# rpp0/gr-lora

Hardware: AMD Instinct MI355X
Metric: IQ Msamples/s demodulated (higher is better)
Workload: dtype f32

## Files before the change

gr_lora_amd/capi.py:

```python
from __future__ import annotations

import ctypes as C
import os
from typing import List, Optional, Sequence, Tuple

import numpy as np

_HERE = os.path.dirname(os.path.abspath(__file__))
LIB_PATH = os.environ.get("LORA_HIP_LIB") or os.path.join(_HERE, "liblora_hip.so")

DEMOD_GRAD, DEMOD_FFT, DEMOD_FFT_COMPAT = 0, 1, 2
FLAG_TRACE = 1
FLAG_PIN_HOST = 2
FLAG_FAST_SYNC = 4
FLAG_NO_DECOUPLED = 8
IQ_CF32, IQ_SC16, IQ_SC8, IQ_CU8 = 0, 1, 2, 3

EXPORTS = [
    "lora_hip_abi_version", "lora_hip_strerror", "lora_hip_last_error", "lora_hip_create", "lora_hip_destroy",
    "lora_hip_get_geometry", "lora_hip_set_sf", "lora_hip_set_samp_rate", "lora_hip_work", "lora_hip_flush",
    "lora_hip_decode_device", "lora_hip_frames_available", "lora_hip_poll_frame", "lora_hip_drain_frames", "lora_hip_drain_slots", "lora_hip_demod_symbols_device", "lora_hip_demod_symbols_ex_device",
    "lora_hip_last_timing", "lora_hip_last_plan", "lora_hip_get_table", "lora_hip_last_payload_pass", "lora_hip_gap_starts_device", "lora_hip_decode_device_begin", "lora_hip_decode_device_end", "lora_hip_decode_device_prepass", "lora_hip_trace", "lora_hip_trace_clear", "lora_hip_check_frame", "lora_hip_estimate_cfo_device", "lora_hip_ref_ifreq_device",
    "lora_hip_set_stream_latency", "lora_hip_stream_info", "lora_hip_stream_info_ex", "lora_hip_walker_kernel_name", "lora_hip_window_stats_device", "lora_hip_detect_preambles_device", "lora_hip_decode_at_headers_device",
    "lora_hip_mux_create", "lora_hip_mux_destroy", "lora_hip_mux_work", "lora_hip_mux_flush", "lora_hip_mux_set_latency", "lora_hip_mux_set_max_ahead", "lora_hip_mux_frames_available",
    "lora_hip_mux_poll_frame", "lora_hip_mux_passes", "lora_hip_mux_last_error",
    "lora_hip_iq_item_bytes", "lora_hip_iq_unpack_device", "lora_hip_work_raw",
]


EXPORTS_CHANNELIZER = [
    "lora_hip_channelizer_create", "lora_hip_channelizer_destroy", "lora_hip_channelizer_last_error", "lora_hip_channelizer_taps",
    "lora_hip_channelizer_output_items", "lora_hip_channelizer_run_device", "lora_hip_channelizer_work", "lora_hip_channelizer_apply_cfo",
    "lora_hip_channelizer_last_kernel_ms", "lora_hip_channelizer_run_device_raw", "lora_hip_channelizer_work_raw",
]


EXPORTS_FILTERBANK = [
    "lora_hip_filterbank_create", "lora_hip_filterbank_destroy", "lora_hip_filterbank_last_error", "lora_hip_filterbank_taps",
    "lora_hip_filterbank_output_items", "lora_hip_filterbank_run_device", "lora_hip_filterbank_run_device_rows", "lora_hip_filterbank_work",
    "lora_hip_filterbank_last_kernel_ms", "lora_hip_filterbank_run_device_raw", "lora_hip_filterbank_run_device_rows_raw", "lora_hip_filterbank_work_raw",
    "lora_hip_filterbank_get_plan",
]


EXPORTS_GATEWAY = [
    "lora_hip_gateway_create", "lora_hip_gateway_destroy", "lora_hip_gateway_last_error", "lora_hip_gateway_work", "lora_hip_gateway_work_device",
    "lora_hip_gateway_flush", "lora_hip_gateway_set_latency", "lora_hip_gateway_frames_available", "lora_hip_gateway_poll_frame", "lora_hip_gateway_stats",
    "lora_hip_gateway_work_raw", "lora_hip_gateway_work_device_raw",
]

EXPORTS_TX = [
    "lora_hip_tx_encode", "lora_hip_tx_frame_items", "lora_hip_tx_create", "lora_hip_tx_destroy", "lora_hip_tx_last_error", "lora_hip_tx_add_frames",
    "lora_hip_tx_generate_device", "lora_hip_tx_generate_device_raw", "lora_hip_tx_generate", "lora_hip_tx_position", "lora_hip_tx_pending",
    "lora_hip_tx_last_kernel_ms",
]

EXPORTS_LINK = [
    "lora_hip_link_measure_device", "lora_hip_link_combine", "lora_hip_link_enable", "lora_hip_link_poll_frame", "lora_hip_link_drain_frames",
    "lora_hip_link_mux_enable", "lora_hip_link_mux_poll_frame", "lora_hip_link_gateway_enable", "lora_hip_link_gateway_poll_frame",
    "lora_hip_link_stats",
]

EXPORTS_SPECTRUM = [
    "lora_hip_spectrum_create", "lora_hip_spectrum_destroy", "lora_hip_spectrum_last_error", "lora_hip_spectrum_window",
    "lora_hip_spectrum_output_rows", "lora_hip_spectrum_run_device", "lora_hip_spectrum_run_device_raw", "lora_hip_spectrum_work",
    "lora_hip_spectrum_work_raw", "lora_hip_spectrum_reset", "lora_hip_spectrum_last_kernel_ms",
]

EXPORTS_RESAMPLER = [
    "lora_hip_resampler_create", "lora_hip_resampler_destroy", "lora_hip_resampler_last_error", "lora_hip_resampler_taps",
    "lora_hip_resampler_ratio", "lora_hip_resampler_delay", "lora_hip_resampler_get_plan", "lora_hip_resampler_output_items",
    "lora_hip_resampler_run_device", "lora_hip_resampler_run_device_raw", "lora_hip_resampler_work", "lora_hip_resampler_work_raw",
    "lora_hip_resampler_reset", "lora_hip_resampler_last_kernel_ms",
]

# ... 124 lines not shown
        d["sync_shift"] = [int(self.sync_shift[0]), int(self.sync_shift[1])]
        return d


class LinkRequest(C.Structure):
    _fields_ = [("stream", C.c_uint32), ("reserved", C.c_uint32), ("header_pos", C.c_int64)]


class LoraHipError(RuntimeError):
    def __init__(self, status: int, msg: str):
        super().__init__("lora_hip status %d: %s" % (status, msg))
        self.status = status


_lib = None


def load():
    global _lib
    if _lib is not None:
        return _lib
    try:
        import torch
    except ImportError:
        pass
    if not os.path.exists(LIB_PATH):
        raise ImportError("liblora_hip.so not built: run `python -c 'import __graft_entry__ as g; g.build()'` "
                          "(hipcc --offload-arch=gfx950).  There is no CPU fallback.")
    L = C.CDLL(LIB_PATH)
    vp = C.c_void_p
    L.lora_hip_abi_version.restype = C.c_uint32
    L.lora_hip_strerror.restype = C.c_char_p
    L.lora_hip_strerror.argtypes = [C.c_int]
    L.lora_hip_last_error.restype = C.c_char_p
    L.lora_hip_last_error.argtypes = [vp]
    L.lora_hip_create.argtypes = [C.POINTER(Config), C.POINTER(vp)]
    L.lora_hip_destroy.argtypes = [vp]
    L.lora_hip_destroy.restype = None
    L.lora_hip_get_geometry.argtypes = [vp, C.POINTER(C.c_uint32), C.POINTER(C.c_uint32), C.POINTER(C.c_uint32)]
    L.lora_hip_set_sf.argtypes = [vp, C.c_uint8]
    L.lora_hip_set_samp_rate.argtypes = [vp, C.c_float]
    L.lora_hip_work.argtypes = [vp, vp, C.c_size_t, C.POINTER(C.c_size_t)]
    L.lora_hip_flush.argtypes = [vp]
    L.lora_hip_decode_device.argtypes = [vp, vp, C.c_size_t, vp, vp, C.c_uint32, vp]
    L.lora_hip_frames_available.restype = C.c_size_t
    L.lora_hip_frames_available.argtypes = [vp]
    L.lora_hip_poll_frame.argtypes = [vp, vp, C.c_size_t, C.POINTER(C.c_size_t), C.POINTER(FrameInfo)]
    L.lora_hip_drain_frames.argtypes = [vp, vp, C.c_size_t, C.POINTER(FrameInfo), C.c_size_t, C.POINTER(C.c_size_t)]
    L.lora_hip_drain_slots.argtypes = [vp, vp, C.c_size_t, C.c_size_t, C.POINTER(C.c_size_t)]
    L.lora_hip_demod_symbols_device.argtypes = [vp, vp, C.c_size_t, vp, C.c_size_t, C.c_int, vp, vp]
    L.lora_hip_demod_symbols_ex_device.argtypes = [vp, vp, C.c_size_t, vp, C.c_size_t, C.c_int, vp, vp, vp]
    L.lora_hip_last_timing.argtypes = [vp, C.POINTER(Timing)]
    L.lora_hip_last_plan.argtypes = [vp, C.POINTER(C.c_uint32), C.POINTER(C.c_uint32)]
    L.lora_hip_last_payload_pass.argtypes = [vp, C.POINTER(C.c_uint32), C.POINTER(C.c_uint32), C.POINTER(C.c_uint32), C.POINTER(C.c_uint32), C.POINTER(C.c_uint32), C.POINTER(C.c_float)]
    L.lora_hip_decode_device_begin.argtypes = [vp, vp, C.c_size_t, vp, vp, C.c_uint32, vp, C.c_uint32]
    L.lora_hip_decode_device_end.argtypes = [vp]
    L.lora_hip_decode_device_prepass.argtypes = [vp, vp, C.c_size_t, vp, vp, C.c_uint32, vp, C.c_uint32]
    L.lora_hip_gap_starts_device.argtypes = [vp, vp, C.c_size_t, vp, vp, C.c_uint32, vp, C.c_size_t, vp, vp]
    L.lora_hip_trace.restype = C.c_size_t
    L.lora_hip_trace.argtypes = [vp, C.POINTER(C.POINTER(Step))]
    L.lora_hip_trace_clear.argtypes = [vp]
    L.lora_hip_trace_clear.restype = None
    L.lora_hip_estimate_cfo_device.argtypes = [vp, vp, C.c_size_t, C.POINTER(C.c_int64), C.c_size_t, C.c_int, C.POINTER(C.c_float), vp]
    L.lora_hip_estimate_cfo_device.restype = C.c_int
    L.lora_hip_ref_ifreq_device.argtypes = [vp, vp, C.c_size_t, C.POINTER(C.c_float), C.POINTER(C.c_float), vp]
    L.lora_hip_ref_ifreq_device.restype = C.c_int
    if hasattr(L, "lora_hip_get_table") or not os.environ.get("LORA_HIP_LIB"):
        L.lora_hip_get_table.argtypes = [vp, C.c_int, C.POINTER(C.c_float), C.c_size_t, C.POINTER(C.c_size_t)]
        L.lora_hip_get_table.restype = C.c_int
    L.lora_hip_window_stats_device.argtypes = [vp, vp, C.c_size_t, vp, C.c_size_t, C.POINTER(WindowStats), vp]
    L.lora_hip_detect_preambles_device.argtypes = [vp, vp, C.c_size_t, vp, vp, C.c_uint32, C.c_float, C.POINTER(Preamble), C.c_size_t, C.POINTER(C.c_size_t), vp]
    L.lora_hip_decode_at_headers_device.argtypes = [vp, vp, C.c_size_t, vp, vp, C.c_uint32, C.POINTER(Preamble), C.c_size_t, vp]
    L.lora_hip_walker_kernel_name.argtypes = [vp]
    L.lora_hip_walker_kernel_name.restype = C.c_char_p
    L.lora_hip_mux_create.argtypes = [C.POINTER(Config), C.c_uint32, C.POINTER(vp)]
    L.lora_hip_mux_destroy.argtypes = [vp]
    L.lora_hip_mux_destroy.restype = None
    L.lora_hip_mux_work.argtypes = [vp, C.c_uint32, vp, C.c_size_t]
    L.lora_hip_mux_flush.argtypes = [vp]
    L.lora_hip_mux_set_latency.argtypes = [vp, C.c_float]
    L.lora_hip_mux_set_max_ahead.argtypes = [vp, C.c_size_t]
    L.lora_hip_mux_frames_available.argtypes = [vp]
    L.lora_hip_mux_frames_available.restype = C.c_size_t
    L.lora_hip_mux_poll_frame.argtypes = [vp, vp, C.c_size_t, C.POINTER(C.c_size_t), C.POINTER(FrameInfo)]
    L.lora_hip_mux_passes.argtypes = [vp, C.POINTER(C.c_uint64), C.POINTER(C.c_uint64)]
    L.lora_hip_mux_last_error.argtypes = [vp]
    L.lora_hip_mux_last_error.restype = C.c_char_p
    L.lora_hip_set_stream_latency.argtypes = [vp, C.c_float]
    L.lora_hip_stream_info.argtypes = [vp, C.POINTER(StreamInfo)]
    if hasattr(L, "lora_hip_stream_info_ex") or not os.environ.get("LORA_HIP_LIB"):
        L.lora_hip_stream_info_ex.argtypes = [vp, C.POINTER(StreamInfo), C.c_uint32]
    L.lora_hip_check_frame.argtypes = [C.c_char_p, C.c_size_t, C.POINTER(FrameCheck)]
    L.lora_hip_check_frame.restype = C.c_int
    L.lora_hip_channelizer_create.argtypes = [C.POINTER(ChannelizerConfig), C.POINTER(vp)]
    L.lora_hip_channelizer_destroy.argtypes = [vp]
    L.lora_hip_channelizer_destroy.restype = None
    L.lora_hip_channelizer_last_error.argtypes = [vp]
    L.lora_hip_channelizer_last_error.restype = C.c_char_p
    L.lora_hip_channelizer_taps.argtypes = [vp, vp, C.c_size_t, C.POINTER(C.c_size_t)]
    L.lora_hip_channelizer_output_items.argtypes = [vp, C.c_size_t]
    L.lora_hip_channelizer_output_items.restype = C.c_size_t
    L.lora_hip_channelizer_run_device.argtypes = [vp, vp, C.c_size_t, vp, C.c_size_t, C.POINTER(C.c_size_t), vp]
    L.lora_hip_channelizer_work.argtypes = [vp, vp, C.c_size_t, vp, C.c_size_t, C.POINTER(C.c_size_t)]
    L.lora_hip_channelizer_apply_cfo.argtypes = [vp, C.c_float]
    L.lora_hip_channelizer_last_kernel_ms.argtypes = [vp]
    L.lora_hip_channelizer_last_kernel_ms.restype = C.c_float
# ... 339 lines not shown
        arr = (LinkRequest * max(n, 1))()
        for i, (st, hp) in enumerate(requests):
            arr[i].stream, arr[i].header_pos = int(st), int(hp)
        mets = (LinkMetrics * max(n, 1))()
        wins = (LinkWindow * max(6 * n, 1))() if windows else None
        self._check(self.L.lora_hip_link_measure_device(self.h, dev_ptr, total_items, o.ctypes.data, l.ctypes.data, o.size, arr, n, mets, wins, stream))
        m = [LinkMetrics.from_buffer_copy(mets[i]) for i in range(n)]
        return (m, [LinkWindow.from_buffer_copy(wins[i]) for i in range(6 * n)]) if windows else m

    def link_stats(self) -> dict:
        a, b, c = C.c_uint64(0), C.c_uint64(0), C.c_double(0.0)
        self._check(self.L.lora_hip_link_stats(self.h, C.byref(a), C.byref(b), C.byref(c)))
        return {"launches": int(a.value), "frames": int(b.value), "kernel_ms": float(c.value)}

    INFO_DTYPE = np.dtype([("stream", "<u4"), ("length", "<u4"), ("header_pos", "<i8"), ("end_pos", "<i8")])

    def drain_raw(self):
        bufs, infos = [], []
        while True:
            n_avail = self.frames_available()
            if n_avail == 0:
                break
            k = min(n_avail, 8192)
            buf = np.empty(k * 280, dtype=np.uint8)
            inf = np.empty(k, dtype=self.INFO_DTYPE)
            n = C.c_size_t(0)
            self._check(self.L.lora_hip_drain_frames(self.h, buf.ctypes.data, buf.size, C.cast(inf.ctypes.data, C.POINTER(FrameInfo)), k, C.byref(n)))
            if n.value == 0:
                break
            inf = inf[: n.value]
            bufs.append(buf[: int(inf["length"].sum())])
            infos.append(inf)
        if not bufs:
            return np.empty(0, dtype=np.uint8), np.empty(0, dtype=self.INFO_DTYPE)
        return np.concatenate(bufs), np.concatenate(infos)

    def drain_slots(self, slot_bytes: int) -> np.ndarray:
        n_avail = self.frames_available()
        out = np.empty((max(n_avail, 1), slot_bytes), dtype=np.uint8)
        n = C.c_size_t(0)
        self._check(self.L.lora_hip_drain_slots(self.h, out.ctypes.data, slot_bytes, n_avail, C.byref(n)))
        return out[: n.value]

    def timing(self) -> Timing:
        t = Timing()
        self._check(self.L.lora_hip_last_timing(self.h, C.byref(t)))
        return t

    def plan(self):
        b, n = C.c_uint32(0), C.c_uint32(0)
        self._check(self.L.lora_hip_last_plan(self.h, C.byref(b), C.byref(n)))
        return bool(b.value), int(n.value)

    def table(self, which: int) -> np.ndarray:
        n = C.c_size_t()
        self._check(self.L.lora_hip_get_table(self.h, which, None, 0, C.byref(n)))
        out = np.empty(n.value, np.float32)
        self._check(self.L.lora_hip_get_table(self.h, which, out.ctypes.data_as(C.POINTER(C.c_float)), n.value, C.byref(n)))
        return out

    def payload_pass(self):
        a, mv, b, r, c, m = C.c_uint32(0), C.c_uint32(0), C.c_uint32(0), C.c_uint32(0), C.c_uint32(0), C.c_float(0)
        self._check(self.L.lora_hip_last_payload_pass(self.h, C.byref(a), C.byref(mv), C.byref(b), C.byref(r), C.byref(c), C.byref(m)))
        return dict(packets=int(a.value), moved=int(mv.value), rerun=int(b.value), rounds=int(r.value), symbols=int(c.value), ms=float(m.value))

    def trace(self):
        p = C.POINTER(Step)()
        n = self.L.lora_hip_trace(self.h, C.byref(p))
        return [(p[i].state, p[i].pos, p[i].consumed, p[i].bin, p[i].fine, p[i].value, p[i].stream, p[i].cycles) for i in range(n)]

    def trace_clear(self):
        self.L.lora_hip_trace_clear(self.h)


class Mux:

    def __init__(self, n_channels, samp_rate=1e6, bandwidth=125000, sf=7, implicit=False, cr=4, crc=True, reduced_rate=False,
                 disable_drift_correction=False, device=0, demod=DEMOD_FFT_COMPAT, flags=0, segment_symbols=0, batch_items=0):
        self.L = load()
        cfg = Config(struct_size=C.sizeof(Config), samp_rate=float(samp_rate), bandwidth=int(bandwidth), sf=int(sf), implicit=int(bool(implicit)), cr=int(cr),
                     crc=int(bool(crc)), reduced_rate=int(bool(reduced_rate)), disable_drift_correction=int(bool(disable_drift_correction)), device=int(device),
                     demod=int(demod), flags=int(flags), segment_symbols=int(segment_symbols), batch_items=int(batch_items))
        self.h = C.c_void_p()
        st = self.L.lora_hip_mux_create(C.byref(cfg), int(n_channels), C.byref(self.h))
        if st != 0:
            raise LoraHipError(st, "%s (%s)" % (self.L.lora_hip_strerror(st).decode(), self.L.lora_hip_last_error(None).decode()))
        self.n_channels = int(n_channels)

    def _check(self, st):
        if st != 0:
            raise LoraHipError(st, "%s (%s)" % (self.L.lora_hip_strerror(st).decode(), (self.L.lora_hip_mux_last_error(self.h) or b"").decode()))

    def work(self, channel: int, iq: np.ndarray):
        a = np.ascontiguousarray(iq, dtype=np.complex64)
        self._check(self.L.lora_hip_mux_work(self.h, int(channel), a.ctypes.data, a.size))

    def flush(self):
        self._check(self.L.lora_hip_mux_flush(self.h))

    def set_latency(self, ms: float):
        self._check(self.L.lora_hip_mux_set_latency(self.h, float(ms)))

    def set_max_ahead(self, items: int):
        self._check(self.L.lora_hip_mux_set_max_ahead(self.h, int(items)))

    def passes(self):
# ... 543 lines not shown
```

gr_lora_amd/csrc/lora_device.h:

```cpp
#pragma once
#include <stdint.h>

#if !defined(__HIPCC__) && !defined(HIP_INCLUDE_HIP_HIP_RUNTIME_H)
struct float2 { float x, y; };
#endif

namespace lora_hip {

constexpr int kWG = 256;
constexpr int kMaxBinsPerThread = 16;
constexpr int kMaxFrame = 3 + 255 + 2;
constexpr int kMaxCodewords = 640;

enum DecState : int32_t { kDetect = 0, kSync, kFindSfd, kPause, kDecodeHeader, kDecodePayload, kStop };

enum AttemptStatus : uint32_t {
    kAttemptNone = 0,
    kAttemptFrame = 1,
    kAttemptLostSync = 2,
    kAttemptOutOfData = 3,
    kAttemptAtHeader = 4,
    kAttemptAtSfd = 5,
    kAttemptHeaderOnly = 6
};
struct SkippedPayload {
    uint8_t  phdr[3];
    uint8_t  n_left;
    uint8_t  left[8];
    int32_t  payload_symbols;
};
constexpr float kSfdIllVar = 1.0f / 4096.0f;
constexpr int kMaxSfdRec = 12;

struct DevParams {
    uint32_t sf, nbins, nbins_hdr, sps, decim, log_nbins, delay_after_sync;
    uint32_t implicit, reduced_rate, enable_fine_sync, demod_mode;
    uint32_t ctor_cr, ctor_crc;
    uint32_t use_fast;
    uint32_t fft_groups;
    uint32_t fft_stride;
    uint32_t lds_work_bytes;
    uint32_t ifreq_in_lds_1;
    uint32_t ifreq_in_lds_2;
    float    down_ifreq_avg;
    float    down_ifreq_sd;
    float    down_ifreq_dsum;
    double   sync_a, sync_b;
    uint32_t sync_closed_form;
    uint32_t strict_sync;
    uint32_t samples_per_second;
    uint32_t ffs_on;
    float    ffs_alpha, ffs_jump, ffs_tol;
    const float2 *down;
    const float  *up_ifreq;
    const float  *down_ifreq;
    const float  *up_ifreq_v;
    const float2 *twN;
    const float2 *tws;
    const float  *wave_tabs;
    const float2 *w3_tw;
    const float2 *w3_ctab;
    const float  *team_tabs;
};

struct Job {
    uint64_t stream_off;
    uint64_t stream_len;
    int64_t  start;
    int64_t  scan_limit;
    uint32_t stream_id;
    uint32_t cr_prev;
    uint32_t max_attempts;
    uint32_t stop_at_header;
    int64_t  probe_limit;
    uint32_t start_at_header;
    uint32_t tail_stop_sfd;
};

struct AttemptRec {
    int64_t  start_pos;
    int64_t  trig_pos;
    int64_t  hdr_pos;
    int64_t  end_pos;
    uint32_t status;
    uint32_t npush;
    float    push_tail[4];
    uint32_t cr_prev;
    uint32_t hdr_ambig;
    uint32_t frame_len;
    uint32_t n_symbols;
    int64_t  sfd_pos[kMaxSfdRec];
    uint32_t n_sfd;
    uint8_t  sfd_fails[kMaxSfdRec];
    uint8_t  frame[kMaxFrame + 4];
};

struct JobResult {
    int64_t  final_pos;
    uint32_t n_attempts;
    uint32_t final_cr;
    uint32_t npush;
    float    push_tail[4];
    uint32_t stop_reason;
    uint32_t n_steps;
    uint32_t pad;
    uint32_t cyc[6];
    uint32_t rounds[6];
    int64_t  tail_final_pos;
    uint32_t tail_valid, tail_first_rec, tail_n_attempts, tail_final_cr, tail_npush, tail_stop_reason, tail_pad, tail_rsv;
    float    tail_push_tail[4];
    uint32_t ctl[4];
    uint32_t dbg[6];
};

struct StepRec {
    int32_t  state, consumed;
    int64_t  pos;
    int32_t  bin, fine;
    float    value;
    uint32_t stream;
    uint32_t cycles;
    uint32_t pad;
};

struct LaunchCfg {
    const float2 *iq;
    const Job *jobs;
    JobResult *results;
    AttemptRec *recs;
    uint32_t recs_per_job;
    float *scratch;
    StepRec *trace;
    uint32_t trace_cap;
    uint32_t n_jobs;
    uint32_t *balance;
    uint32_t skip_payload;
};
constexpr uint32_t kBalanceCus = 2048;
constexpr uint32_t kBalanceWords = 3u * kBalanceCus;

struct EnvStream {
    uint64_t off;
    uint32_t first_block;
    uint32_t n_blocks;
};
int launch_envelope(const float2 *iq, const EnvStream *streams , uint32_t n_streams, uint32_t sps,
                    float *d_E, unsigned long long *d_bitmap , void *stream);

int launch_walker(const DevParams &p, const LaunchCfg &c, void *stream);
const char *walker_kernel_name(const DevParams &p);
struct DemodAlt { int32_t *shift; uint32_t *bins; int32_t *fine; int64_t max_start; };
int launch_demod_symbols(const DevParams &p, const float2 *iq, const int64_t *d_offsets, uint32_t n,
                         int demod, uint32_t *d_bins, int32_t *d_fine, float *scratch, void *stream, const DemodAlt *alt = nullptr);
int launch_detect_windows(const DevParams &p, const float2 *iq, const int64_t *d_offsets, uint32_t n, void *d_out , void *stream);
constexpr int kPayloadHyp = 4;
struct PayloadDesc {
    uint32_t n_walk;
    uint32_t n_hyp;
    int32_t  hyp_shift[kPayloadHyp];
    int32_t  hyp_base[kPayloadHyp];
    uint32_t hyp_from[kPayloadHyp];
    uint32_t hyp_to[kPayloadHyp];
    int64_t  room;
    SkippedPayload sk;
};
enum PayloadWalk : uint32_t { kWalkComplete = 0, kWalkOutOfData = 1, kWalkNeedShift = 2 };
struct PayloadOut {
    uint32_t result;
    uint32_t at;
    int32_t  shift;
    uint32_t frame_len;
    uint8_t  frame[kMaxFrame + 4];
};
int launch_payload_chain(const DevParams &p, const uint32_t *d_bins, const int32_t *d_fine, const DemodAlt &alt, const PayloadDesc *descs, PayloadOut *outs, uint32_t n_packets, void *stream);
bool walker_has_skip_variant(const DevParams &p);
int launch_ref_ifreq(const float2 *x, uint32_t n, float *d_arg, float *d_ifreq, void *stream);
int launch_cfo(const DevParams &p, const float2 *iq, const int64_t *d_offsets, uint32_t n, int mode, float *d_out, void *stream);
bool walker3_covers(uint32_t sf);
uint32_t w3_tw_entries(uint32_t sf);
void build_w3_tables(uint32_t sf, float2 *tw, float2 *ctab );
uint32_t wave_tables_floats(uint32_t sf);
void build_wave_tables(uint32_t sf, const float2 *down, float *out);
uint32_t wave_tables_floats_d(uint32_t sf, uint32_t decim);
void build_wave_tables_d(uint32_t sf, uint32_t decim, const float2 *down, float *out);
uint32_t team_tables_entries(uint32_t sf);
void build_team_tables(uint32_t sf, const float2 *down, double dt, double bandwidth, float2 *out);
uint32_t walker_lds_bytes(const DevParams &p);
uint32_t walker_resident_slots(const DevParams &p);
uint32_t walker_resident_slots_full(const DevParams &p);
const char *walker_kernel_name_for(const DevParams &p, uint32_t n_jobs, bool skip = false);

}
```

gr_lora_amd/csrc/lora_kernels.hip:

```cpp

#include <hip/hip_runtime.h>
#include <math.h>
#include <stdio.h>
#include <atomic>
#include <cstdlib>
#include <stdint.h>
#include <type_traits>

#include "lora_device.h"
#include "whitening_data.inc"

namespace lora_hip {

__constant__ unsigned char c_whiten_cr56[LORA_WHITEN_CR56_LEN];
__constant__ unsigned char c_whiten_cr78[LORA_WHITEN_CR78_LEN];
__constant__ unsigned char c_h84_decode[256];
static std::atomic<bool> g_consts_ready[16];

static unsigned char h_hamming_encode(unsigned v)
{
    const unsigned b0 = v & 1u, b1 = (v >> 1) & 1u, b2 = (v >> 2) & 1u, b3 = (v >> 3) & 1u;
    const unsigned p1 = b1 ^ b2 ^ b3, p2 = b0 ^ b1 ^ b2, p3 = b0 ^ b1 ^ b3, p4 = b0 ^ b2 ^ b3;
    return (unsigned char)(p1 | (b0 << 1) | (b1 << 2) | (b2 << 3) | (p2 << 4) | (b3 << 5) | (p3 << 6) | (p4 << 7));
}
// ... 291 lines not shown
constexpr int brev_bits(int v, int bits)
{
    int r = 0;
    for (int b = 0; b < bits; b++) if (v & (1 << b)) r |= 1 << (bits - 1 - b);
    return r;
}
constexpr int ilog2(int v) { return v <= 1 ? 0 : 1 + ilog2(v >> 1); }

#define LORA_DPP(old, v, ctrl, bank) __builtin_amdgcn_update_dpp((old), (v), (ctrl), 0xf, (bank), false)

template <int MASK>
__device__ __forceinline__ float lane_xor(float f)
{
    const int v = __builtin_bit_cast(int, f);
    int r;
    if constexpr (MASK == 1) r = LORA_DPP(0, v, 0xB1, 0xf);
    else if constexpr (MASK == 2) r = LORA_DPP(0, v, 0x4E, 0xf);
    else if constexpr (MASK == 4) {
        r = LORA_DPP(0, v, 0x104, 0x5);
        r = LORA_DPP(r, v, 0x114, 0xA);
    } else if constexpr (MASK == 8) r = LORA_DPP(0, v, 0x128, 0xf);
    else if constexpr (MASK == 16) {
        const auto p = __builtin_amdgcn_permlane16_swap(v, v, false, false);
        r = (threadIdx.x & 16) ? p[0] : p[1];
    } else {
        const auto p = __builtin_amdgcn_permlane32_swap(v, v, false, false);
        r = (threadIdx.x & 32) ? p[0] : p[1];
    }
    return __builtin_bit_cast(float, r);
}

template <int MASK>
__device__ __forceinline__ float2 lane_xor2(float2 v) { return make_float2(lane_xor<MASK>(v.x), lane_xor<MASK>(v.y)); }

__device__ __forceinline__ float wave_sum_rows(float v)
{
    v += lane_xor<1>(v); v += lane_xor<2>(v); v += lane_xor<4>(v); v += lane_xor<8>(v);
    const float r0 = __builtin_bit_cast(float, __builtin_amdgcn_readlane(__builtin_bit_cast(int, v), 0));
    const float r1 = __builtin_bit_cast(float, __builtin_amdgcn_readlane(__builtin_bit_cast(int, v), 16));
    const float r2 = __builtin_bit_cast(float, __builtin_amdgcn_readlane(__builtin_bit_cast(int, v), 32));
    const float r3 = __builtin_bit_cast(float, __builtin_amdgcn_readlane(__builtin_bit_cast(int, v), 48));
    return (r0 + r1) + (r2 + r3);
}

__device__ __forceinline__ uint32_t uni32(uint32_t v) { return (uint32_t)__builtin_amdgcn_readfirstlane((int)v); }
__device__ __forceinline__ uint64_t uni64(uint64_t v) { return ((uint64_t)uni32((uint32_t)(v >> 32)) << 32) | uni32((uint32_t)v); }
__device__ __forceinline__ Job uniform_job(const Job &j)
{
    Job u;
    u.stream_off = uni64(j.stream_off); u.stream_len = uni64(j.stream_len);
    u.start = (int64_t)uni64((uint64_t)j.start); u.scan_limit = (int64_t)uni64((uint64_t)j.scan_limit);
    u.stream_id = uni32(j.stream_id); u.cr_prev = uni32(j.cr_prev); u.max_attempts = uni32(j.max_attempts); u.stop_at_header = uni32(j.stop_at_header);
    u.probe_limit = (int64_t)uni64((uint64_t)j.probe_limit);
    u.start_at_header = uni32(j.start_at_header); u.tail_stop_sfd = uni32(j.tail_stop_sfd);
    return u;
}

__device__ __forceinline__ uint32_t rotl_bits(uint32_t bits, uint32_t count, uint32_t size)
{
    const uint32_t mask = (1u << size) - 1u;
    count %= size;
    bits &= mask;
    return ((bits << count) & mask) | (bits >> (size - count));
}

__device__ __forceinline__ uint8_t deshuffle_byte(uint8_t v)
{
    return (uint8_t)(((v >> 5) & 1u) | (((v >> 0) & 1u) << 1) | (((v >> 1) & 1u) << 2) | (((v >> 2) & 1u) << 3) |
                     (((v >> 4) & 1u) << 4) | (((v >> 3) & 1u) << 5) | (((v >> 6) & 1u) << 6) | (((v >> 7) & 1u) << 7));
}

__device__ __forceinline__ uint8_t data_bits(uint8_t cw)
{
    return (uint8_t)(((cw >> 1) & 1u) | (((cw >> 2) & 1u) << 1) | (((cw >> 3) & 1u) << 2) | (((cw >> 5) & 1u) << 3));
}

__device__ void deinterleave_block(Shared &sh, uint32_t n_words, uint32_t ppm, uint32_t &n_cw)
{
    if (n_words <= 8u) {
        uint32_t r[8];
#pragma unroll
        for (uint32_t i = 0; i < 8u; i++) r[i] = (i < n_words) ? rotl_bits(sh.words[i], i, ppm) : 0u;
        for (uint32_t x = 0; x < ppm; x++) {
            uint32_t c = 0;
#pragma unroll
            for (uint32_t i = 0; i < 8u; i++) c |= ((r[i] >> x) & 1u) << i;
            if (n_cw < kMaxCodewords) sh.cw[n_cw++] = (uint8_t)c;
        }
        return;
    }
    for (uint32_t x = 0; x < ppm; x++) {
        uint8_t c = 0;
        for (uint32_t i = 0; i < n_words; i++) c |= (uint8_t)(((rotl_bits(sh.words[i], i, ppm) >> x) & 1u) << i);
        if (n_cw < kMaxCodewords) sh.cw[n_cw++] = c;
    }
}
__device__ __forceinline__ void deinterleave_block_wave(Shared &sh, uint64_t words_pk, uint32_t n_words, uint32_t ppm, uint32_t &n_cw)
{
    const uint32_t lane = threadIdx.x & 63u, x = lane >> 3, i = lane & 7u;
    const uint32_t w = (uint32_t)(words_pk >> (8u * i)) & 0xffu;
    int sh_amt = (int)x - (int)(i % ppm);
    if (sh_amt < 0) sh_amt += (int)ppm;
    const bool bit = x < ppm && i < n_words && ((w >> sh_amt) & 1u);
    const unsigned long long m = __ballot(bit);
    if (i == 0u && x < ppm && n_cw + x < (uint32_t)kMaxCodewords) sh.cw[n_cw + x] = (uint8_t)((m >> (8u * x)) & 0xffu);
    n_cw = (n_cw + ppm <= (uint32_t)kMaxCodewords) ? n_cw + ppm : (uint32_t)kMaxCodewords;
}
// ... 507 lines not shown
    __syncthreads();
    for (uint32_t t = lane; t < n_blocks * ppm; t += blockDim.x) {
        const uint32_t b = t / ppm, x = t - b * ppm;
        uint32_t c = 0;
        for (uint32_t i = 0; i < B; i++) c |= ((rotl_bits(words[b * B + i], i, ppm) >> x) & 1u) << i;
        if (n_left + t < (uint32_t)kMaxCodewords) sh.cw[n_left + t] = (uint8_t)c;
    }
    const uint32_t n_cw = (n_left + n_blocks * ppm <= (uint32_t)kMaxCodewords) ? n_left + n_blocks * ppm : (uint32_t)kMaxCodewords;
    uint32_t n_bytes;
    if (cr >= 3u) n_bytes = (uint32_t)ceilf((float)n_cw * 4.0f / (4.0f + (float)cr));
    else n_bytes = (n_cw + 1u) / 2u;
    if (n_bytes > (uint32_t)(kMaxCodewords / 2 + 8)) n_bytes = kMaxCodewords / 2 + 8;
    const uint32_t payload_length = (uint32_t)d.sk.phdr[0] + 2u * has_crc;
    const uint32_t plen = payload_length > 257u ? 257u : payload_length;
    decode_payload_bytes(sh, n_cw, cr, n_bytes);
    for (uint32_t i = lane; i < plen; i += blockDim.x) o.frame[3u + i] = (i < n_bytes) ? sh.dec[i] : 0;
    if (lane == 0) {
        o.frame[0] = d.sk.phdr[0]; o.frame[1] = d.sk.phdr[1]; o.frame[2] = d.sk.phdr[2];
        o.frame_len = 3u + plen;
    }
}

#include "lora_detect.inc.hip"

static bool use_fast_kernel(const DevParams &p)
{
    return p.use_fast && p.decim == 8u && (p.sf == 7u || p.sf == 8u) && (p.demod_mode == 0u || p.wave_tabs);
}

static bool use_fast_decim(const DevParams &p)
{
    return p.use_fast && walker2_decim_covers(p.sf, p.decim) && (p.demod_mode == 0u || p.wave_tabs);
}

static bool use_w3_kernel(const DevParams &p)
{
    return p.use_fast && p.decim == 8u && walker3_covers(p.sf) && p.w3_tw && p.w3_ctab;
}

struct WalkerKernel {
    void (*fn)(DevParams, LaunchCfg);
    uint32_t threads, lds;
    const char *name = "walker_kernel";
};

static bool w3_has_half(const DevParams &p) { return p.use_fast && p.decim == 8u && ((p.sf == 9u && p.demod_mode == 0u) || p.sf == 10u) && p.w3_tw && p.w3_ctab; }
static int w3_half_policy()
{
    static const int pol = getenv("LORA_HIP_W3_HALF") ? atoi(getenv("LORA_HIP_W3_HALF")) : -1;
    return pol;
}

bool walker_has_skip_variant(const DevParams &p) { return (use_w3_kernel(p) || use_fast_kernel(p)) && !p.implicit; }

static WalkerKernel pick_walker(const DevParams &p, bool half = false, bool skip = false)
{
    if (skip && walker_has_skip_variant(p) && use_fast_kernel(p)) {
        const bool g = p.demod_mode == 0u;
        if (p.sf == 7u) return {g ? walker2_kernel_sf7_grad_skip : walker2_kernel_sf7_skip, walker2_threads(7), walker2_lds_bytes(7, g), g ? "walker2_kernel_sf7_grad_skip" : "walker2_kernel_sf7_skip"};
        return {g ? walker2_kernel_sf8_grad_skip : walker2_kernel_sf8_skip, walker2_threads(8), walker2_lds_bytes(8, g), g ? "walker2_kernel_sf8_grad_skip" : "walker2_kernel_sf8_skip"};
    }
    if (skip && walker_has_skip_variant(p)) {
        void (*fn)(DevParams, LaunchCfg);
        if (p.demod_mode == 0u) fn = p.sf == 9u ? walker3_kernel_sf9_grad_skip : p.sf == 10u ? walker3_kernel_sf10_grad_skip : p.sf == 11u ? walker3_kernel_sf11_grad_skip : walker3_kernel_sf12_grad_skip;
        else fn = p.sf == 9u ? walker3_kernel_sf9_skip : p.sf == 10u ? walker3_kernel_sf10_skip : p.sf == 11u ? walker3_kernel_sf11_skip : walker3_kernel_sf12_skip;
        static const char *const names[2][4] = {{"walker3_kernel_sf9_skip", "walker3_kernel_sf10_skip", "walker3_kernel_sf11_skip", "walker3_kernel_sf12_skip"},
                                                 {"walker3_kernel_sf9_grad_skip", "walker3_kernel_sf10_grad_skip", "walker3_kernel_sf11_grad_skip", "walker3_kernel_sf12_grad_skip"}};
        return {fn, walker3_threads(p.sf), walker3_lds(p.sf), names[p.demod_mode == 0u ? 1 : 0][p.sf - 9u]};
    }
    if (use_fast_kernel(p)) {
        if (p.demod_mode == 0u) {
            if (p.sf == 7u) return {walker2_kernel_sf7_grad, walker2_threads(7), walker2_lds_bytes(7, true), "walker2_kernel_sf7_grad"};
            return {walker2_kernel_sf8_grad, walker2_threads(8), walker2_lds_bytes(8, true), "walker2_kernel_sf8_grad"};
        }
        if (p.sf == 7u) return {walker2_kernel_sf7, walker2_threads(7), walker2_lds_bytes(7), "walker2_kernel_sf7"};
        return {walker2_kernel_sf8, walker2_threads(8), walker2_lds_bytes(8), "walker2_kernel_sf8"};
    }
    if (use_fast_decim(p)) {
        const bool g = p.demod_mode == 0u;
        const uint32_t lds = walker2_lds_bytes(p.sf, g, p.decim);
        if (p.sf == 6u && p.decim == 8u) return {g ? walker2_kernel_sf6_d8_grad : walker2_kernel_sf6_d8, 512u, lds, g ? "walker2_kernel_sf6_d8_grad" : "walker2_kernel_sf6_d8"};
        if (p.sf == 6u) return {g ? walker2_kernel_sf6_d4_grad : walker2_kernel_sf6_d4, 512u, lds, g ? "walker2_kernel_sf6_d4_grad" : "walker2_kernel_sf6_d4"};
        if (p.sf == 7u && p.decim == 2u) return {g ? walker2_kernel_sf7_d2_grad : walker2_kernel_sf7_d2, 512u, lds, g ? "walker2_kernel_sf7_d2_grad" : "walker2_kernel_sf7_d2"};
        if (p.sf == 7u) return {g ? walker2_kernel_sf7_d4_grad : walker2_kernel_sf7_d4, 512u, lds, g ? "walker2_kernel_sf7_d4_grad" : "walker2_kernel_sf7_d4"};
        if (p.sf == 9u && p.decim == 2u) return {g ? walker2_kernel_sf9_d2_grad : walker2_kernel_sf9_d2, 512u, lds, g ? "walker2_kernel_sf9_d2_grad" : "walker2_kernel_sf9_d2"};
        if (p.sf == 9u) return {g ? walker2_kernel_sf9_d4_grad : walker2_kernel_sf9_d4, 512u, lds, g ? "walker2_kernel_sf9_d4_grad" : "walker2_kernel_sf9_d4"};
        if (p.decim == 2u) return {g ? walker2_kernel_sf8_d2_grad : walker2_kernel_sf8_d2, 512u, lds, g ? "walker2_kernel_sf8_d2_grad" : "walker2_kernel_sf8_d2"};
        return {g ? walker2_kernel_sf8_d4_grad : walker2_kernel_sf8_d4, 512u, lds, g ? "walker2_kernel_sf8_d4_grad" : "walker2_kernel_sf8_d4"};
    }
    if (use_w3_kernel(p) && half && w3_has_half(p)) {
        if (p.demod_mode == 0u) return {p.sf == 9u ? walker3_kernel_sf9_grad_half : walker3_kernel_sf10_grad_half, walker3_threads_half(p.sf), walker3_lds_half(p.sf),
                                        p.sf == 9u ? "walker3_kernel_sf9_grad_half" : "walker3_kernel_sf10_grad_half"};
        return {walker3_kernel_sf10_half, walker3_threads_half(p.sf), walker3_lds_half(p.sf), "walker3_kernel_sf10_half"};
    }
    if (use_w3_kernel(p)) {
        void (*fn)(DevParams, LaunchCfg);
        if (p.demod_mode == 0u) fn = p.sf == 9u ? walker3_kernel_sf9_grad : p.sf == 10u ? walker3_kernel_sf10_grad : p.sf == 11u ? walker3_kernel_sf11_grad : walker3_kernel_sf12_grad;
        else fn = p.sf == 9u ? walker3_kernel_sf9 : p.sf == 10u ? walker3_kernel_sf10 : p.sf == 11u ? walker3_kernel_sf11 : walker3_kernel_sf12;
        static const char *const names[2][4] = {{"walker3_kernel_sf9", "walker3_kernel_sf10", "walker3_kernel_sf11", "walker3_kernel_sf12"},
                                                 {"walker3_kernel_sf9_grad", "walker3_kernel_sf10_grad", "walker3_kernel_sf11_grad", "walker3_kernel_sf12_grad"}};
        return {fn, walker3_threads(p.sf), walker3_lds(p.sf), names[p.demod_mode == 0u ? 1 : 0][p.sf - 9u]};
    }
    const uint32_t b = (p.lds_work_bytes + (uint32_t)sizeof(Shared) + 15u) & ~15u;
    if (p.ifreq_in_lds_2) return {walker_kernel, (uint32_t)kWG, b, "walker_kernel"};
    if (p.ifreq_in_lds_1) return {walker_kernel_f1, (uint32_t)kWG, b, "walker_kernel_f1"};
    return {walker_kernel_f0, (uint32_t)kWG, b, "walker_kernel_f0"};
// ... 327 lines not shown
```

gr_lora_amd/csrc/lora_runtime.cpp:

```cpp

#include <hip/hip_runtime.h>

#include <algorithm>
#include <cmath>
#include <cstddef>
#include <cstdarg>
#include <cstdio>
#include <cstdlib>
#include <cstring>
#include <chrono>
#include <deque>
#include <new>
#include <string>
#include <vector>

#include "../../include/lora_hip.h"
#include "../../include/lora_hip_link.h"
#include "lora_device.h"
#include "lora_link.h"
#include "lora_stitch.hpp"
#include "lora_mux_dev.h"
#include "lora_iq.h"

using namespace lora_hip;
// ... 62 lines not shown
        hipError_t e = hipMalloc((void **)&p, want * sizeof(T));
        if (e == hipSuccess) cap = want;
        return e;
    }
    void release() { if (p) (void)hipFree(p); p = nullptr; cap = 0; }
};

struct ChunkPipe {
    struct Chan : StreamCarry {
        size_t fill = 0;
    };
    std::vector<Chan> ch;
    DevBuf<float2> dbuf[2];
    int cur = 0;
    size_t batch = 0, tailcap = 0, region = 0;
    hipStream_t copy_st = nullptr, comp_st = nullptr;
    hipEvent_t up_ev = nullptr, tail_ev = nullptr;
    bool inflight = false;
    float max_latency_ms = 50.0f;
    std::chrono::steady_clock::time_point t_first;
    bool have_first = false;
    uint64_t passes = 0, passes_by_latency = 0;
    float2 *row(size_t c) const { return dbuf[cur].p + c * region + tailcap + ch[c].fill; }
};

}

struct lora_hip_decoder {
    lora_hip_config_t cfg{};
    DevParams P{};
    int device = 0;
    float2 *d_down = nullptr, *d_twN = nullptr, *d_tws = nullptr;
    float *d_wave_tabs = nullptr;
    float2 *d_w3_tw = nullptr, *d_w3_ctab = nullptr;
    float2 *d_team_tabs = nullptr;
    float *d_up_ifreq = nullptr, *d_down_ifreq = nullptr, *d_up_ifreq_v = nullptr;
    std::vector<float2> h_up;
    size_t n_up_ifreq_v = 0;
    DevBuf<Job> d_jobs;
    DevBuf<JobResult> d_results;
    DevBuf<AttemptRec> d_recs;
    DevBuf<float> d_scratch;
    DevBuf<StepRec> d_trace;
    DevBuf<float2> d_staging;
    DevBuf<int64_t> d_offsets;
    DevBuf<uint32_t> d_bins;
    RunOut run_out[2];
    std::vector<JobResult> h_results;
    std::vector<AttemptRec> h_recs;
    std::vector<StepRec> h_trace;
    hipEvent_t ev0 = nullptr, ev1 = nullptr, ev_done = nullptr;
    hipEvent_t ev_pre0 = nullptr, ev_pre1 = nullptr, ev_dep = nullptr;
    hipStream_t pre_stream = nullptr;
    struct Pending { uint32_t nj = 0, recs_per_job = 0, eager = 0, trace_cap = 0; bool direct = true, open = false; hipStream_t st = nullptr;
                     std::chrono::steady_clock::time_point hp0, hp1; } pending;
    PassCtx pass;
    std::vector<StreamDesc> pass_streams;
    int64_t resume_pos = 0;
    uint32_t resume_cr = 0;
    const float2 *pass_iq = nullptr;
    hipStream_t pass_st = nullptr;
    bool pass_open = false, iq_ready = false;
    bool pre_issued = false;
    const float2 *pre_iq = nullptr;
    uint64_t pre_sig = 0;
    uint32_t pre_ns = 0;
    std::chrono::steady_clock::time_point pre_hq0;
    FrameQueue frames;
    PinnedBuf<Job> p_jobs;
    PinnedBuf<JobResult> p_res;
    PinnedBuf<AttemptRec> p_recs;
    DevBuf<uint32_t> d_balance;
    DevBuf<float> d_env_E;
    DevBuf<unsigned long long> d_env_buf;
    PinnedBuf<EnvStream> p_env_streams;
    PinnedBuf<unsigned long long> p_env_buf;
    float envelope_ms = 0.0f;
    std::vector<lora_hip_step_t> trace;
    lora_hip_timing_t timing{};
    std::string err;
    ChunkPipe pipe;
    struct HostFeed {
        PinnedBuf<float2> stage[2];
        hipEvent_t stage_ev[2] = {nullptr, nullptr};
        bool stage_busy[2] = {false, false};
        int stage_i = 0;
        DevBuf<uint32_t> d_raw;
        std::vector<std::pair<uintptr_t, uintptr_t>> pinned;
        std::vector<std::pair<uintptr_t, uintptr_t>> refused;
    } feed;
    const char *last_kernel = nullptr;
    uint32_t last_kernel_jobs = 0;
    uint32_t resident_slots = 0;
    uint32_t resident_slots_alt = ~0u;
    uint32_t eager_recs = 4;
    uint32_t last_plan_burst = 0, last_plan_segments = 0;
    int decoupled_policy = -1;
    bool launch_skip = false;
    uint32_t dec_backoff = 0;
    uint32_t last_payload_packets = 0, last_payload_rerun = 0, last_payload_symbols = 0, last_payload_moved = 0, last_payload_rounds = 0;
    float last_payload_ms = 0.0f;
    PinnedBuf<int64_t> p_pay_off;
    PinnedBuf<PayloadDesc> p_pay_desc;
    PinnedBuf<PayloadOut> p_pay_out;
    DevBuf<int32_t> d_fine, d_alt_shift, d_alt_fine;
    DevBuf<uint32_t> d_alt_bins;
    hipStream_t pay_stream = nullptr;
    hipEvent_t ev_pay0 = nullptr, ev_pay1 = nullptr, ev_pay_done = nullptr;
    struct Link {
        struct Pending { size_t ref; uint64_t off, len; int64_t hdr_pos; };
        bool on = false;
        float *d_hann = nullptr;
        DevBuf<LinkWindowDesc> d_wins;
        DevBuf<LinkWindowRec> d_recs;
        std::vector<LinkWindowDesc> h_wins;
        std::vector<lora_hip_link_window_t> h_recs;
        std::vector<Pending> pending;
        hipEvent_t ev0 = nullptr, ev1 = nullptr;
        uint64_t launches = 0, frames = 0;
        double kernel_ms = 0.0;
    } link;
    struct PayState { std::vector<uint32_t> active; size_t used = 0, cap_sym = 0, n_sym = 0; int round = 0; float ms = 0.0f; bool open = false; } pay;
};

namespace {
// ... 185 lines not shown
void publish(lora_hip_decoder *h, const AttemptRec &r, StreamDesc &sd)
{
    lora_hip_frame_info_t info;
    info.stream = sd.id;
    info.length = (uint32_t)kLoratapLen + r.frame_len;
    info.header_pos = sd.abs_base + r.hdr_pos;
    info.end_pos = sd.abs_base + r.end_pos;
    uint8_t *blob = h->frames.push(info.length, info);
    blob[13] = snr_byte(sd.pwr.snr);
    std::memcpy(blob + kLoratapLen, r.frame, r.frame_len);
    if (h->link.on) h->link.pending.push_back({h->frames.refs.size() - 1u, sd.off, sd.len, r.hdr_pos});
}

lora_hip_status run_jobs_begin(lora_hip_decoder *h, const float2 *d_iq, const std::vector<Job> &jobs, uint32_t recs_per_job,
                               uint32_t trace_cap, hipStream_t st, RunOut &out)
{
    const uint32_t nj = (uint32_t)jobs.size();
    const auto hp0 = std::chrono::steady_clock::now();
    if (h->pending.open) return fail(h, LORA_HIP_ERR_INTERNAL, "a launch is already in flight on this handle");
    h->pending = lora_hip_decoder::Pending{};
    h->pending.nj = nj; h->pending.recs_per_job = recs_per_job; h->pending.trace_cap = trace_cap; h->pending.st = st; h->pending.hp0 = hp0;
    out.rpj = recs_per_job; out.cap = recs_per_job;
    out.res.resize(nj);
    out.recs.clear();
    if (nj == 0) return LORA_HIP_OK;
    static const bool staged_bufs = getenv("LORA_HIP_STAGED") != nullptr;
    if (staged_bufs) {
        HIP_TRY(h, h->d_jobs.reserve(nj));
        HIP_TRY(h, h->d_results.reserve(nj));
        HIP_TRY(h, h->d_recs.reserve((size_t)nj * recs_per_job));
    }
    const bool need_scratch = !h->P.ifreq_in_lds_2;
    if (need_scratch) HIP_TRY(h, h->d_scratch.reserve((size_t)nj * 2u * h->P.sps));
    if (trace_cap) HIP_TRY(h, h->d_trace.reserve((size_t)nj * trace_cap));
    static const bool direct = getenv("LORA_HIP_STAGED") == nullptr;
    const uint32_t eager = direct ? recs_per_job : std::min(std::max(h->eager_recs, 2u), recs_per_job);
    HIP_TRY(h, h->p_jobs.reserve(nj));
    HIP_TRY(h, h->p_res.reserve(nj));
    HIP_TRY(h, h->p_recs.reserve((size_t)nj * eager));
    std::memcpy(h->p_jobs.p, jobs.data(), nj * sizeof(Job));
    if (!direct) HIP_TRY(h, hipMemcpyAsync(h->d_jobs.p, h->p_jobs.p, nj * sizeof(Job), hipMemcpyHostToDevice, st));
    LaunchCfg c{};
    c.iq = d_iq; c.recs_per_job = recs_per_job;
    c.jobs = direct ? h->p_jobs.p : h->d_jobs.p; c.results = direct ? h->p_res.p : h->d_results.p; c.recs = direct ? h->p_recs.p : h->d_recs.p;
    c.scratch = need_scratch ? h->d_scratch.p : nullptr;
    c.trace = trace_cap ? h->d_trace.p : nullptr; c.trace_cap = trace_cap; c.n_jobs = nj;
    static const bool no_balance = getenv("LORA_HIP_NO_BALANCE") != nullptr;
    if (!h->d_balance.p && !no_balance) {
        HIP_TRY(h, h->d_balance.reserve(kBalanceWords));
        HIP_TRY(h, hipMemsetAsync(h->d_balance.p, 0, kBalanceWords * sizeof(uint32_t), st));
    }
    c.balance = no_balance ? nullptr : h->d_balance.p;
    c.skip_payload = h->launch_skip ? 1u : 0u;
    HIP_TRY(h, hipEventRecord(h->ev0, st));
    if (nj >= h->last_kernel_jobs) { h->last_kernel = walker_kernel_name_for(h->P, nj, h->launch_skip); h->last_kernel_jobs = nj; }
    if (launch_walker(h->P, c, st) != 0) return fail(h, LORA_HIP_ERR_HIP, "walker launch failed: %s", hipGetErrorString(hipGetLastError()));
    HIP_TRY(h, hipEventRecord(h->ev1, st));
    if (!direct) {
        HIP_TRY(h, hipMemcpyAsync(h->p_res.p, h->d_results.p, nj * sizeof(JobResult), hipMemcpyDeviceToHost, st));
        HIP_TRY(h, hipMemcpy2DAsync(h->p_recs.p, eager * sizeof(AttemptRec), h->d_recs.p, recs_per_job * sizeof(AttemptRec), eager * sizeof(AttemptRec), nj,
                                    hipMemcpyDeviceToHost, st));
    }
    HIP_TRY(h, hipEventRecord(h->ev_done, st));
    h->pending.eager = eager; h->pending.direct = direct; h->pending.open = true;
    h->pending.hp1 = std::chrono::steady_clock::now();
    return LORA_HIP_OK;
}

lora_hip_status run_jobs_end(lora_hip_decoder *h, RunOut &out)
{
    if (!h->pending.open) return LORA_HIP_OK;
    h->pending.open = false;
    const uint32_t nj = h->pending.nj, recs_per_job = h->pending.recs_per_job, eager = h->pending.eager, trace_cap = h->pending.trace_cap;
    const hipStream_t st = h->pending.st;
    const auto hp0 = h->pending.hp0, hp1 = h->pending.hp1;
    const Job *jobs = h->p_jobs.p;
    HIP_TRY(h, hipEventSynchronize(h->ev_done));
    const auto hp2 = std::chrono::steady_clock::now();
    std::memcpy(out.res.data(), h->p_res.p, nj * sizeof(JobResult));
    static const bool dbg_stats = getenv("LORA_HIP_DEBUG") != nullptr;
    if (dbg_stats && h->P.use_fast) {
        double cyc[6] = {0}, rnd[6] = {0};
        for (uint32_t j = 0; j < nj; j++) for (int i = 0; i < 6; i++) { cyc[i] += 64.0 * out.res[j].cyc[i]; rnd[i] += out.res[j].rounds[i]; }
        fprintf(stderr, "[lora_hip] per-job avg kcycles (rounds): DETECT %.0f (%.1f) SYNC %.0f (%.1f) SFD %.0f (%.1f) PAUSE %.0f (%.1f) HDR %.0f (%.1f) PAYLOAD %.0f (%.1f)\n",
                cyc[0] / nj / 1e3, rnd[0] / nj, cyc[1] / nj / 1e3, rnd[1] / nj, cyc[2] / nj / 1e3, rnd[2] / nj, cyc[3] / nj / 1e3, rnd[3] / nj, cyc[4] / nj / 1e3, rnd[4] / nj, cyc[5] / nj / 1e3, rnd[5] / nj);
        {
            double na = 0, nt = 0, ntv = 0; uint32_t sr[4] = {0, 0, 0, 0}, tsr[4] = {0, 0, 0, 0}, tpad = 0;
            for (uint32_t j = 0; j < nj; j++) {
                const JobResult &r = out.res[j];
                na += r.n_attempts; sr[r.stop_reason & 3u]++;
                if (r.tail_valid) { ntv++; nt += r.tail_n_attempts; tsr[r.tail_stop_reason & 3u]++; tpad += r.tail_pad; }
            }
            fprintf(stderr, "[lora_hip] attempts/job %.2f, stop reasons %u/%u/%u/%u; tails %.0f (attempts/tail %.2f, stop reasons %u/%u/%u/%u, pending %u)\n", na / nj, sr[0], sr[1],
                    sr[2], sr[3], ntv, ntv ? nt / ntv : 0.0, tsr[0], tsr[1], tsr[2], tsr[3], tpad);
        }
        double ctl[4] = {0};
        for (uint32_t j = 0; j < nj; j++) for (int i = 0; i < 4; i++) ctl[i] += 64.0 * out.res[j].ctl[i];
        fprintf(stderr, "[lora_hip] control per job, kcycles: copy-in %.0f loop %.0f plan %.0f copy-out %.0f (walker3: demodulation %.0f, replay %.0f of the decode rounds; with LORA_W3_REPLAY_STATS=2 copy-in and symbol loop in the 3rd / 4th figure)\n", ctl[0] / nj / 1e3, ctl[1] / nj / 1e3, ctl[2] / nj / 1e3, ctl[3] / nj / 1e3, ctl[0] / nj / 1e3, ctl[1] / nj / 1e3);
        std::vector<double> tot(nj);
        for (uint32_t j = 0; j < nj; j++) { double t = 0; for (int i = 0; i < 6; i++) t += 64.0 * out.res[j].cyc[i]; tot[j] = t; }
        std::sort(tot.begin(), tot.end());
        double mean = 0; for (double t : tot) mean += t; mean /= nj;
        fprintf(stderr, "[lora_hip] job kcycles over %u jobs: min %.0f p50 %.0f p90 %.0f max %.0f mean %.0f\n", nj, tot[0] / 1e3, tot[nj / 2] / 1e3,
                tot[(size_t)(nj * 0.9)] / 1e3, tot[nj - 1] / 1e3, mean / 1e3);
    }
    if (const char *tl = getenv("LORA_HIP_JOB_TIMELINE")) {
        if (FILE *f = fopen(tl, "a")) {
            fprintf(f, "# launch of %u jobs: job hw_id xcc_id t_start t_end(100MHz) cyc[6] x64 start scan_limit n_att\n", nj);
            for (uint32_t j = 0; j < nj; j++) {
                const JobResult &r = out.res[j];
                fprintf(f, "%u %u %u %u %u %u %u %u %u %u %u %lld %lld %u %u %u %u %u\n", j, r.dbg[0], r.dbg[1], r.dbg[2], r.dbg[3], r.cyc[0], r.cyc[1], r.cyc[2], r.cyc[3], r.cyc[4], r.cyc[5],
                        (long long)jobs[j].start, (long long)jobs[j].scan_limit, r.n_attempts, r.dbg[5] - r.dbg[4], r.rounds[5], r.rounds[0], r.rounds[2]);
            }
            fclose(f);
        }
    }
    uint32_t max_att = 0;
    for (uint32_t j = 0; j < nj; j++) max_att = std::max(max_att, out.res[j].n_attempts + (out.res[j].tail_valid ? out.res[j].tail_n_attempts : 0u));
    if (max_att > recs_per_job) max_att = recs_per_job;
    const uint32_t stride = std::max(max_att, 1u);
    out.rpj = stride;
    out.recs.resize_uninit((size_t)nj * stride);
    for (uint32_t j = 0; j < nj; j++) {
        const uint32_t used = std::min(std::min(eager, max_att), out.res[j].n_attempts + (out.res[j].tail_valid ? out.res[j].tail_n_attempts : 0u));
        for (uint32_t a = 0; a < used; a++) {
            const AttemptRec *src = h->p_recs.p + (size_t)j * eager + a;
            const size_t n = offsetof(AttemptRec, frame) + std::min<size_t>(src->frame_len, sizeof src->frame);
            std::memcpy(&out.recs[(size_t)j * stride + a], src, n);
        }
    }
    if (dbg_stats && h->P.use_fast) {
        double sync_rounds = 0; uint32_t frames = 0, tails = 0, early = 0;
        for (uint32_t j = 0; j < nj; j++) {
            const JobResult &r = out.res[j];
            sync_rounds += r.rounds[1];
            const uint32_t used = std::min(std::min(eager, max_att), r.n_attempts + (r.tail_valid ? r.tail_n_attempts : 0u));
            for (uint32_t a = 0; a < used; a++) {
                const AttemptRec &t = out.recs[(size_t)j * stride + a];
                frames += (a < r.n_attempts && t.status == kAttemptFrame) ? 1u : 0u;
                if (r.tail_valid && a + 1u == r.n_attempts + r.tail_n_attempts && r.tail_pad) { tails++; early += t.status == kAttemptAtSfd ? 1u : 0u; }
            }
        }
        fprintf(stderr, "[lora_hip] acquisitions: %.0f SYNC rounds for %u frames of this launch (%.2f per frame); %u tail probes reached a packet, %u of them stopped behind their first FIND_SFD step\n",
                sync_rounds, frames, frames ? sync_rounds / frames : 0.0, tails, early);
    }
    h->eager_recs = std::min(std::max(max_att, 2u), 8u);
    bool more = false;
    if (max_att > eager) {
        HIP_TRY(h, hipMemcpy2DAsync(out.recs.data() + eager, stride * sizeof(AttemptRec), h->d_recs.p + eager,
                                    recs_per_job * sizeof(AttemptRec), (max_att - eager) * sizeof(AttemptRec), nj, hipMemcpyDeviceToHost, st));
        more = true;
    }
    if (trace_cap) {
        h->h_trace.resize((size_t)nj * trace_cap);
        HIP_TRY(h, hipMemcpyAsync(h->h_trace.data(), h->d_trace.p, (size_t)nj * trace_cap * sizeof(StepRec), hipMemcpyDeviceToHost, st));
        more = true;
    }
    if (more) HIP_TRY(h, hipStreamSynchronize(st));
    float ms = 0.0f;
    HIP_TRY(h, hipEventElapsedTime(&ms, h->ev0, h->ev1));
    if (dbg_stats) {
        const auto hp3 = std::chrono::steady_clock::now();
        auto us = [](auto a, auto b) { return std::chrono::duration<double, std::micro>(b - a).count(); };
        fprintf(stderr, "[lora_hip] run_jobs host: enqueue %.0f us, wait %.0f us (kernel %.0f us), unpack %.0f us; results %zu B + records %zu B\n", us(hp0, hp1), us(hp1, hp2),
                ms * 1e3, us(hp2, hp3), nj * sizeof(JobResult), (size_t)nj * eager * sizeof(AttemptRec));
    }
    h->timing.walker_ms += ms;
    h->timing.total_device_ms += ms;
    h->timing.walker_launches++;
    return LORA_HIP_OK;
}

lora_hip_status run_jobs(lora_hip_decoder *h, const float2 *d_iq, const std::vector<Job> &jobs, uint32_t recs_per_job, uint32_t trace_cap,
                         hipStream_t st, RunOut &out)
{
    const lora_hip_status s = run_jobs_begin(h, d_iq, jobs, recs_per_job, trace_cap, st, out);
    return s == LORA_HIP_OK ? run_jobs_end(h, out) : s;
}

void append_trace(lora_hip_decoder *h, const RunOut &out, uint32_t job_index, uint32_t trace_cap, int64_t abs_base)
{
    const JobResult &jr = out.res[job_index];
    for (uint32_t i = 0; i < jr.n_steps; i++) {
        const StepRec &s = h->h_trace[(size_t)job_index * trace_cap + i];
        lora_hip_step_t o;
        o.state = s.state; o.consumed = s.consumed; o.pos = abs_base + s.pos; o.bin = s.bin; o.fine = s.fine;
        o.value = s.value; o.stream = s.stream; o.cycles = s.cycles; o.reserved = 0;
        h->trace.push_back(o);
    }
}

uint64_t streams_signature(const std::vector<StreamDesc> &streams)
{
    uint64_t x = 1469598103934665603ull;
    for (const StreamDesc &sd : streams)
        for (uint64_t v : {sd.off, sd.len}) { x ^= v; x *= 1099511628211ull; }
    return x ^ streams.size();
// ... 215 lines not shown
    uint32_t ctor_cr() const { return h->P.ctor_cr; }
    uint32_t segment_symbols() const { return h->cfg.segment_symbols; }
    uint32_t resident_slots() const
    {
        if (h->resident_slots == 0) h->resident_slots = std::max<uint32_t>(walker_resident_slots(h->P), 64u);
        return h->resident_slots;
    }
    uint32_t resident_slots_alt() const
    {
        if (h->resident_slots_alt == ~0u) h->resident_slots_alt = walker_resident_slots_full(h->P);
        return h->resident_slots_alt;
    }
    bool tracing() const { return (h->cfg.flags & LORA_HIP_FLAG_TRACE) != 0; }
    bool implicit() const { return h->P.implicit != 0; }
    bool early_probe() const
    {
        static const bool off = getenv("LORA_HIP_NO_EARLY_PROBE") != nullptr;
        return !off && h->P.use_fast && h->P.decim == 8u && walker3_covers(h->P.sf);
    }
    bool decoupled(size_t n_jobs)
    {
        h->last_payload_packets = 0; h->last_payload_rerun = 0; h->last_payload_symbols = 0; h->last_payload_ms = 0.0f; h->last_payload_moved = 0; h->last_payload_rounds = 0;
        if (h->decoupled_policy == 0 || !walker_has_skip_variant(h->P) || tracing()) return false;
        if (h->decoupled_policy == 1) return true;
        if (h->dec_backoff) return false;
        const uint32_t full = resident_slots_alt() ? resident_slots_alt() : resident_slots();
        constexpr uint32_t fill = 100u;
        return 100u * (uint32_t)n_jobs <= fill * full;
    }
    void set_skip_payload(bool on) { h->launch_skip = on; }
    void abort_payload() { ::payload_pass_abort(h); }
    int run_payload_begin(std::vector<PayloadReq> &reqs) { return ::payload_pass_begin(h, d_iq, reqs) == LORA_HIP_OK ? 0 : -1; }
    int run_payload_end(std::vector<PayloadReq> &reqs) { return ::payload_pass_end(h, d_iq, reqs) == LORA_HIP_OK ? 0 : -1; }
    void count_payload(uint32_t packets, uint32_t moved, uint32_t rerun)
    {
        h->last_payload_packets += packets; h->last_payload_rerun += rerun; h->last_payload_moved += moved;
        if (rerun) h->timing.slow_path_relaunches++;
        if (h->decoupled_policy < 0 && packets >= 4u && 4u * (rerun + moved) > packets) h->dec_backoff = 32;
        static const bool dbg = getenv("LORA_HIP_DEBUG") != nullptr;
        if (dbg) fprintf(stderr, "[lora_hip] payload pass: %u packets, %u symbol reads in %u round(s), %.3f ms; %u packet(s) ended off the zero-drift grid (their jobs split there), %u handed to the complete kernels\n",
                         packets, h->last_payload_symbols, h->last_payload_rounds, h->last_payload_ms, moved, rerun);
    }
    RunOut &run_out(int which) { return h->run_out[which & 1]; }
    bool quiet_edges(const std::vector<StreamDesc> &streams, std::vector<std::vector<int64_t>> &edges)
    {
        return ::quiet_edges(h, d_iq, streams, st, edges) == LORA_HIP_OK;
    }
    int run_jobs(const std::vector<Job> &jobs, uint32_t rpj, uint32_t trace_cap, RunOut &out)
    {
        return ::run_jobs(h, d_iq, jobs, rpj, trace_cap, st, out) == LORA_HIP_OK ? 0 : -1;
    }
    int run_jobs_begin(const std::vector<Job> &jobs, uint32_t rpj, uint32_t trace_cap, RunOut &out)
    {
        return ::run_jobs_begin(h, d_iq, jobs, rpj, trace_cap, st, out) == LORA_HIP_OK ? 0 : -1;
    }
    int run_jobs_end(RunOut &out) { return ::run_jobs_end(h, out) == LORA_HIP_OK ? 0 : -1; }
    void publish(const AttemptRec &r, StreamDesc &sd) { ::publish(h, r, sd); }
    void append_trace(const RunOut &out, uint32_t job, uint32_t cap, int64_t base) { ::append_trace(h, out, job, cap, base); }
    void count_jobs(uint32_t n) { h->timing.jobs += n; h->last_kernel_jobs = 0; if (h->dec_backoff) h->dec_backoff--; }
    void count_probes(uint32_t n) { h->timing.probes += n; }
    void count_slow_path() { h->timing.slow_path_relaunches++; }
    void count_repair()
    {
        static const bool dbg = getenv("LORA_HIP_DEBUG") != nullptr;
        if (dbg) fprintf(stderr, "[lora_hip] cut repaired from the true header (no serial walk)\n");
    }
    void note_plan(bool burst_aware, size_t n_segs)
    {
        h->last_plan_burst = burst_aware ? 1u : 0u; h->last_plan_segments = (uint32_t)n_segs;
        static const bool dbg = getenv("LORA_HIP_DEBUG") != nullptr;
        if (dbg) fprintf(stderr, "[lora_hip] segment plan: %s, %zu segments (envelope kernels %.3f ms)\n", burst_aware ? "burst-aware" : "fixed grid", n_segs, burst_aware ? h->envelope_ms : 0.0f);
    }
    double walker_ms() const { return h->timing.walker_ms; }
};

constexpr double kLinkNorm = 0.375 * 2.0;

void link_combine(const lora_hip_link_window_t *w, uint32_t sps, uint32_t nbins, double bandwidth, lora_hip_link_metrics_t *out)
{
    *out = lora_hip_link_metrics_t{};
    const double N = (double)nbins, D = (double)sps / N, norm = kLinkNorm * (double)sps * (double)sps;
    auto wrap = [N](double v) { v = std::fmod(v + 0.5 * N, N); if (v < 0.0) v += N; return v - 0.5 * N; };
    bool pair[3];
    double pos[6] = {0, 0, 0, 0, 0, 0}, mid[3] = {0, 0, 0};
    for (int p = 0; p < 3; p++) {
        pair[p] = w[2 * p].valid != 0u && w[2 * p + 1].valid != 0u;
        if (!pair[p]) continue;
        out->flags |= 1u << p;
        for (int k = 0; k < 2; k++) pos[2 * p + k] = wrap((double)w[2 * p + k].peak_bin + (double)w[2 * p + k].frac);
        mid[p] = wrap(pos[2 * p] + 0.5 * wrap(pos[2 * p + 1] - pos[2 * p]));
    }
    double s_sum = 0.0, nb_sum = 0.0;
    int cnt = 0;
    for (int p = 0; p < 3; p += 2) {
        if (!pair[p]) continue;
        for (int k = 0; k < 2; k++) {
            const lora_hip_link_window_t &x = w[2 * p + k];
            const double nb = std::max(((double)x.total_power - (double)x.lobe_power) / (N - 7.0), 0.0);
            s_sum += std::max((double)x.lobe_power - 7.0 * nb, 0.0);
            nb_sum += nb;
            cnt++;
        }
    }
    out->rssi_dbfs = out->snr_db = LORA_HIP_LINK_FLOOR_DB;
    if (cnt) {
        out->signal_power = s_sum / cnt / norm;
// ... 261 lines not shown
    if (cfg->sf < 6 || cfg->sf > 12) return LORA_HIP_ERR_BAD_SF;
    if (cfg->cr > 4 || cfg->demod < 0 || cfg->demod > 2 || cfg->bandwidth == 0 || !(cfg->samp_rate >= 1.0f)) return LORA_HIP_ERR_BAD_CONFIG;
    int ndev = 0;
    const hipError_t ec = hipGetDeviceCount(&ndev);
    if (ec != hipSuccess || ndev <= 0 || cfg->device < 0 || cfg->device >= ndev)
        return fail(nullptr, LORA_HIP_ERR_NO_DEVICE, "hipGetDeviceCount: %s, %d device(s), requested %d", hipGetErrorString(ec), ndev, cfg->device);
    lora_hip_decoder *h = new (std::nothrow) lora_hip_decoder();
    if (!h) return LORA_HIP_ERR_NOMEM;
    h->cfg = *cfg;
    h->device = cfg->device;
    lora_hip_status s = LORA_HIP_OK;
    const hipError_t es = hipSetDevice(h->device);
    if (es != hipSuccess) s = fail(nullptr, LORA_HIP_ERR_NO_DEVICE, "hipSetDevice(%d): %s", h->device, hipGetErrorString(es));
    if (s == LORA_HIP_OK) s = build_tables(h);
    if (s == LORA_HIP_OK && (hipEventCreate(&h->ev0) != hipSuccess || hipEventCreate(&h->ev1) != hipSuccess || hipEventCreate(&h->ev_done) != hipSuccess ||
                             hipEventCreate(&h->ev_pre0) != hipSuccess || hipEventCreate(&h->ev_pre1) != hipSuccess ||
                             hipEventCreateWithFlags(&h->ev_dep, hipEventDisableTiming) != hipSuccess ||
                             hipStreamCreateWithFlags(&h->pre_stream, hipStreamNonBlocking) != hipSuccess ||
                             hipStreamCreateWithFlags(&h->pay_stream, hipStreamNonBlocking) != hipSuccess || hipEventCreate(&h->ev_pay0) != hipSuccess ||
                             hipEventCreate(&h->ev_pay1) != hipSuccess || hipEventCreate(&h->ev_pay_done) != hipSuccess))
        s = LORA_HIP_ERR_HIP;
    if (s != LORA_HIP_OK) { lora_hip_destroy(h); return s; }
    pipe_init(h, 1, cfg->batch_items ? cfg->batch_items : std::max<size_t>(1u << 20, 64ull * h->P.sps));
    *out = h;
    return LORA_HIP_OK;
}

void lora_hip_destroy(lora_hip_decoder_t *h)
{
    if (!h) return;
    (void)hipSetDevice(h->device);
    if (h->pipe.comp_st) { (void)hipStreamSynchronize(h->pipe.copy_st); (void)hipStreamSynchronize(h->pipe.comp_st); }
    if (h->d_down) (void)hipFree(h->d_down);
    if (h->d_twN) (void)hipFree(h->d_twN);
    if (h->d_tws) (void)hipFree(h->d_tws);
    if (h->d_wave_tabs) (void)hipFree(h->d_wave_tabs);
    if (h->d_w3_tw) (void)hipFree(h->d_w3_tw);
    if (h->d_team_tabs) (void)hipFree(h->d_team_tabs);
    if (h->d_w3_ctab) (void)hipFree(h->d_w3_ctab);
    if (h->d_up_ifreq) (void)hipFree(h->d_up_ifreq);
    if (h->d_down_ifreq) (void)hipFree(h->d_down_ifreq);
    if (h->d_up_ifreq_v) (void)hipFree(h->d_up_ifreq_v);
    if (h->link.d_hann) (void)hipFree(h->link.d_hann);
    h->link.d_wins.release(); h->link.d_recs.release();
    for (hipEvent_t e : {h->link.ev0, h->link.ev1})
        if (e) (void)hipEventDestroy(e);
    h->p_pay_off.release(); h->p_pay_desc.release(); h->p_pay_out.release(); h->d_fine.release(); h->d_alt_shift.release(); h->d_alt_bins.release(); h->d_alt_fine.release();
    h->d_jobs.release(); h->d_results.release(); h->d_recs.release(); h->d_scratch.release();
    h->d_trace.release(); h->d_staging.release(); h->d_offsets.release(); h->d_bins.release();
    for (auto &r : h->feed.pinned) (void)hipHostUnregister((void *)r.first);
    for (int i = 0; i < 2; i++) { h->pipe.dbuf[i].release(); h->feed.stage[i].release(); }
    h->feed.d_raw.release();
    h->p_jobs.release(); h->p_res.release(); h->p_recs.release();
    h->d_balance.release(); h->d_env_E.release(); h->d_env_buf.release(); h->p_env_streams.release(); h->p_env_buf.release();
    for (hipEvent_t e : {h->ev0, h->ev1, h->ev_done, h->ev_pre0, h->ev_pre1, h->ev_dep, h->ev_pay0, h->ev_pay1, h->ev_pay_done, h->pipe.up_ev, h->pipe.tail_ev,
                         h->feed.stage_ev[0], h->feed.stage_ev[1]})
        if (e) (void)hipEventDestroy(e);
    for (hipStream_t st : {h->pre_stream, h->pay_stream, h->pipe.copy_st, h->pipe.comp_st})
        if (st) (void)hipStreamDestroy(st);
    delete h;
}

lora_hip_status lora_hip_get_table(const lora_hip_decoder_t *h, int which, float *buf, size_t cap_floats, size_t *n_floats)
{
    if (!h) return LORA_HIP_ERR_ARG;
    const size_t sps = h->P.sps;
    const void *src = nullptr;
    size_t n = 0;
    bool on_device = true;
    switch (which) {
    case 0: src = h->d_down; n = 2 * sps; break;
    case 1: src = h->h_up.data(); n = 2 * sps; on_device = false; break;
    case 2: src = h->d_down_ifreq; n = sps; break;
    case 3: src = h->d_up_ifreq; n = sps; break;
    case 4: src = h->d_up_ifreq_v; n = h->n_up_ifreq_v; break;
    default: return LORA_HIP_ERR_ARG;
    }
    if (n_floats) *n_floats = n;
    if (!buf) return LORA_HIP_OK;
    if (cap_floats < n || !src) return LORA_HIP_ERR_ARG;
    if (!on_device) { memcpy(buf, src, n * sizeof(float)); return LORA_HIP_OK; }
    if (hipSetDevice(h->device) != hipSuccess || hipMemcpy(buf, src, n * sizeof(float), hipMemcpyDeviceToHost) != hipSuccess) return LORA_HIP_ERR_HIP;
    return LORA_HIP_OK;
}

lora_hip_status lora_hip_get_geometry(const lora_hip_decoder_t *h, uint32_t *sps, uint32_t *bins, uint32_t *decim)
{
    if (!h) return LORA_HIP_ERR_ARG;
    if (sps) *sps = h->P.sps;
    if (bins) *bins = h->P.nbins;
    if (decim) *decim = h->P.decim;
    return LORA_HIP_OK;
}

lora_hip_status lora_hip_set_sf(lora_hip_decoder_t *h, uint8_t sf)
{
    if (!h) return LORA_HIP_ERR_ARG;
    (void)sf;
    fprintf(stderr, "[LoRa Decoder] WARNING : Setting the spreading factor during execution is currently not supported.\n"
                    "Nothing set, kept SF of %u.\n", (unsigned)h->P.sf);
    return LORA_HIP_OK;
}

lora_hip_status lora_hip_set_samp_rate(lora_hip_decoder_t *h, float samp_rate)
{
    if (!h) return LORA_HIP_ERR_ARG;
// ... 723 lines not shown
            o.header_pos = c.a0 + delta + found * sps + 2 * sps + sps / 4; o.run_pos = c.k * sps; o.stream = c.stream; o.run_len = (uint32_t)(c.e - c.k);
            o.bin = c.bin; o.sfd_index = (int32_t)found; o.pmr = c.pmr; o.cfo_bins = -0.5f * (float)sb;
            o.cfo_hz = o.cfo_bins * (float)h->cfg.bandwidth / (float)N; o.delta = (int32_t)delta;
        } else overflow = true;
        n_out++;
    }
    *n_found = n_out;
    return overflow ? LORA_HIP_ERR_OVERFLOW : LORA_HIP_OK;
}

lora_hip_status lora_hip_decode_at_headers_device(lora_hip_decoder_t *h, const void *d_iq, size_t total_items, const uint64_t *stream_off,
                                                  const uint64_t *stream_len, uint32_t n_streams, const lora_hip_preamble_t *pre, size_t n, void *hip_stream)
{
    if (!h || !d_iq || !n_streams || !stream_off || !stream_len || (n && !pre)) return LORA_HIP_ERR_ARG;
    if (h->pass_open) return fail(h, LORA_HIP_ERR_ARG, "lora_hip_decode_at_headers_device: a pass is open on this handle");
    if (h->P.implicit) return fail(h, LORA_HIP_ERR_BAD_CONFIG, "decode at given headers needs an explicit header (the implicit mode's energy threshold comes from DETECT)");
    if (n == 0) return LORA_HIP_OK;
    HIP_TRY(h, hipSetDevice(h->device));
    std::vector<Job> jobs(n, Job{});
    for (size_t i = 0; i < n; i++) {
        const uint32_t s = pre[i].stream;
        if (s >= n_streams || stream_off[s] > total_items || stream_len[s] > total_items - stream_off[s]) return fail(h, LORA_HIP_ERR_ARG, "entry %zu: bad stream", i);
        if (pre[i].header_pos < 0 || (uint64_t)pre[i].header_pos + 2u * h->P.sps > stream_len[s]) return fail(h, LORA_HIP_ERR_ARG, "entry %zu: header position outside its stream", i);
        Job &j = jobs[i];
        j.stream_off = stream_off[s]; j.stream_len = stream_len[s]; j.stream_id = s;
        j.start = pre[i].header_pos; j.scan_limit = pre[i].header_pos;
        j.cr_prev = h->P.ctor_cr; j.max_attempts = 1; j.start_at_header = 1;
    }
    h->err.clear();
    h->timing = lora_hip_timing_t{};
    RunOut &out = h->run_out[0];
    const lora_hip_status rc = run_jobs(h, (const float2 *)d_iq, jobs, 2, 0, (hipStream_t)hip_stream, out);
    if (rc != LORA_HIP_OK) return rc;
    for (size_t i = 0; i < n; i++) {
        if (out.res[i].n_attempts == 0 || out.rpj == 0) continue;
        const AttemptRec &r = out.rec(i, 0);
        if (r.status != kAttemptFrame) continue;
        StreamDesc sd{};
        sd.id = jobs[i].stream_id; sd.abs_base = 0;
        sd.off = jobs[i].stream_off; sd.len = jobs[i].stream_len;
        publish(h, r, sd);
    }
    return h->link.pending.empty() ? LORA_HIP_OK : link_measure_pending(h, (const float2 *)d_iq, (hipStream_t)hip_stream);
}

lora_hip_status lora_hip_last_plan(const lora_hip_decoder_t *h, uint32_t *burst_aware, uint32_t *segments)
{
    if (!h) return LORA_HIP_ERR_ARG;
    if (burst_aware) *burst_aware = h->last_plan_burst;
    if (segments) *segments = h->last_plan_segments;
    return LORA_HIP_OK;
}

lora_hip_status lora_hip_last_payload_pass(const lora_hip_decoder_t *h, uint32_t *packets, uint32_t *moved, uint32_t *rerun, uint32_t *rounds, uint32_t *symbols, float *ms)
{
    if (!h) return LORA_HIP_ERR_ARG;
    if (packets) *packets = h->last_payload_packets;
    if (moved) *moved = h->last_payload_moved;
    if (rounds) *rounds = h->last_payload_rounds;
    if (rerun) *rerun = h->last_payload_rerun;
    if (symbols) *symbols = h->last_payload_symbols;
    if (ms) *ms = h->last_payload_ms;
    return LORA_HIP_OK;
}

const char *lora_hip_walker_kernel_name(const lora_hip_decoder_t *h) { return h ? (h->last_kernel ? h->last_kernel : walker_kernel_name(h->P)) : ""; }

lora_hip_status lora_hip_last_timing(const lora_hip_decoder_t *h, lora_hip_timing_t *t)
{
    if (!h || !t) return LORA_HIP_ERR_ARG;
    *t = h->timing;
    return LORA_HIP_OK;
}

size_t lora_hip_trace(const lora_hip_decoder_t *h, const lora_hip_step_t **steps)
{
    if (!h || !steps) return 0;
    *steps = h->trace.data();
    return h->trace.size();
}

void lora_hip_trace_clear(lora_hip_decoder_t *h)
{
    if (h) h->trace.clear();
}

lora_hip_status lora_hip_link_combine(const lora_hip_link_window_t *windows, uint32_t sps, uint32_t nbins, double bandwidth, lora_hip_link_metrics_t *out)
{
    if (!windows || !out || nbins < 16u || sps < nbins || (sps & (sps - 1u)) != 0u || (nbins & (nbins - 1u)) != 0u) return LORA_HIP_ERR_ARG;
    link_combine(windows, sps, nbins, bandwidth, out);
    return LORA_HIP_OK;
}

lora_hip_status lora_hip_link_measure_device(lora_hip_decoder_t *h, const void *d_iq, size_t total_items, const uint64_t *stream_off,
                                             const uint64_t *stream_len, uint32_t n_streams, const lora_hip_link_request_t *req, size_t n,
                                             lora_hip_link_metrics_t *metrics_out, lora_hip_link_window_t *windows_out, void *hip_stream)
{
    if (!h || !d_iq || !n_streams || !stream_off || !stream_len || (n && (!req || !metrics_out))) return LORA_HIP_ERR_ARG;
    if (h->pass_open) return fail(h, LORA_HIP_ERR_ARG, "lora_hip_link_measure_device: a pass is open on this handle");
    for (uint32_t s = 0; s < n_streams; s++)
        if (stream_off[s] > total_items || stream_len[s] > total_items - stream_off[s]) return fail(h, LORA_HIP_ERR_ARG, "stream %u exceeds the buffer", s);
    std::vector<LinkReq> rq(n);
    for (size_t i = 0; i < n; i++) {
        if (req[i].stream >= n_streams) return fail(h, LORA_HIP_ERR_ARG, "request %zu: bad stream", i);
        rq[i] = LinkReq{stream_off[req[i].stream], stream_len[req[i].stream], req[i].header_pos};
    }
// ... 60 lines not shown
```

gr_lora_amd/csrc/lora_stitch.hpp:

```cpp
#pragma once
#include <algorithm>
#include <chrono>
#include <cstdint>
#include <cstdio>
#include <cstdlib>
#include <cstring>
#include <memory>
#include <vector>

#include "lora_device.h"

namespace lora_hip {

struct PwrState {
    float q[4];
    int n = 0;
    float snr = 0.0f;
    void push(float v)
    {
        if (n < 4) q[n++] = v;
        else { q[0] = q[1]; q[1] = q[2]; q[2] = q[3]; q[3] = v; }
    }
    void apply(uint32_t npush, const float tail[4])
    {
// ... 154 lines not shown
template <class Env>
int run_serial(Env &env, StreamDesc &sd, Cursor &cur, int64_t limit, bool tracing)
{
    while (true) {
        const std::vector<Job> jobs(1, walk_job(sd, cur, limit, false));
        const uint64_t span = (uint64_t)std::max<int64_t>(limit - cur.pos, 0);
        const uint32_t rpj = recs_for(span, env.sps());
        const uint32_t trace_cap = tracing ? (uint32_t)std::min<uint64_t>(2ull * (span / env.sps()) + 64ull, 1ull << 22) : 0u;
        RunOut out;
        int s = env.run_jobs(jobs, rpj, trace_cap, out);
        if (s != 0) return s;
        const JobResult &jr = out.res[0];
        if (debug_jobs_on()) dump_job("serial", 0, jobs[0], out);
        if (!end_known(out, 0)) {
            if (debug_on()) fprintf(stderr, "[lora_hip] serial walk of stream %u from %lld: %u attempts, the pending one's record did not fit %u records - the decode fails\n",
                                    sd.id, (long long)cur.pos, jr.n_attempts, out.cap);
            return -1;
        }
        for (uint32_t a = 0; a < out.n_done(0); a++) adopt(env, out.rec(0, a), sd);
        if (tracing) env.append_trace(out, 0, trace_cap, sd.abs_base);
        cur = end_cursor(out, 0);
        if (jr.pad) { sd.incomplete = true; return 0; }
        sd.pwr.apply(jr.npush, jr.push_tail);
        if (jr.stop_reason != 2u) return 0;
    }
}

inline int cr_class(uint32_t cr) { return cr >= 3u ? 2 : (cr >= 1u ? 1 : 0); }

inline bool wrong_fec_branch(const AttemptRec &r, uint32_t true_cr)
{
    const int cj = cr_class(r.cr_prev), cl = cr_class(true_cr);
    return cj != cl && (r.hdr_ambig || cj == 0 || cl == 0);
}

inline bool header_bearing(const AttemptRec &r, bool with_header_only)
{
    return r.hdr_pos >= 0 && (r.status == kAttemptFrame || r.status == kAttemptOutOfData || (with_header_only && r.status == kAttemptHeaderOnly));
}

inline bool passed_sfd_state(const AttemptRec &r, int64_t pos, uint32_t fails)
{
    for (uint32_t z = 0; z < r.n_sfd && z < (uint32_t)kMaxSfdRec; z++)
        if (r.sfd_pos[z] == pos && r.sfd_fails[z] == fails) return true;
    return false;
}

inline const AttemptRec *tail_probe_last(const RunOut &R, size_t k)
{
    const JobResult &jr = R.res[k];
    if (!jr.tail_valid || !jr.tail_pad || jr.tail_n_attempts == 0u) return nullptr;
    const uint32_t li = std::min(jr.tail_first_rec, R.cap) + jr.tail_n_attempts - 1u;
    return li < R.cap ? &R.rec(k, li) : nullptr;
}

template <class Pred>
int find_record(const RunOut &R, size_t k, Pred pred)
{
    const uint32_t nall = std::min(R.res[k].n_attempts, R.cap);
    for (uint32_t a = 0; a < nall; a++)
        if (pred(R.rec(k, a))) return (int)a;
    return -1;
}

template <class Pred>
bool any_segment_record(const RunOut &R, size_t first, size_t target, Pred pred)
{
    for (size_t k = first + 1; k <= target; k++)
        if (find_record(R, k, [&](const AttemptRec &r) { return header_bearing(r, true) && pred(r); }) >= 0) return true;
    return false;
}

inline bool plan_burst_segments(const std::vector<StreamDesc> &streams, const std::vector<std::vector<int64_t>> &edges, uint32_t sps,
                                uint32_t slots, uint64_t nominal, std::vector<std::vector<int64_t>> &cuts)
{
    if (edges.size() != streams.size() || slots == 0) return false;
    size_t n_edges = 0;
    for (const auto &e : edges) n_edges += e.size();
    if (n_edges < slots) return false;
    const int64_t acq = 40ll * sps;
    auto weight = [&](const std::vector<int64_t> &e, size_t k, int64_t len) {
        const int64_t a = k ? e[k - 1] : 0;
        return k < e.size() ? (e[k] - a) + acq : len - a;
    };
    double total = 0;
    for (size_t i = 0; i < streams.size(); i++)
        for (size_t k = 0; k <= edges[i].size(); k++) total += (double)weight(edges[i], k, (int64_t)streams[i].len);
    double target = total / slots;
    for (int attempt = 0; attempt < 12; attempt++, target *= 1.07) {
        size_t n_segs = 0;
        cuts.assign(streams.size(), {});
        for (size_t i = 0; i < streams.size(); i++) {
            const std::vector<int64_t> &e = edges[i];
            const int64_t len = (int64_t)streams[i].len;
            double acc = 0;
            for (size_t k = 0; k < e.size(); k++) {
                acc += (double)weight(e, k, len);
                if (acc >= target - 0.5 * (double)weight(e, k + 1, len) && len - e[k] > 8ll * sps && e[k] > (cuts[i].empty() ? 0 : cuts[i].back())) {
                    cuts[i].push_back(e[k]);
                    acc = 0;
                }
            }
            std::vector<int64_t> c;
            int64_t prev = 0;
            for (size_t k = 0; k <= cuts[i].size(); k++) {
                const int64_t b = k < cuts[i].size() ? cuts[i][k] : len;
// ... 75 lines not shown
                    planned = env.decoupled(n_segs);
                    if (!planned) cuts.clear();
                }
            }
            if (!planned) balanced = planned = plan_burst_segments(streams, edges, sps, slots, seg, cuts);
            const uint32_t alt = env.resident_slots_alt();
            if (!planned && alt && alt < slots) {
                const uint64_t seg_alt = std::max<uint64_t>(64ull * sps, (total + alt - alt / 16u - 1) / (alt - alt / 16u));
                balanced = planned = plan_burst_segments(streams, edges, sps, alt, seg_alt, cuts);
            }
        }
    }

    if (!planned && segmenting && env.segment_symbols() == 0 && env.resident_slots_alt() && env.resident_slots_alt() < slots) {
        const uint32_t alt = env.resident_slots_alt();
        const uint64_t wj = std::max<uint64_t>(alt - alt / 16u, (uint64_t)streams.size());
        seg = std::max<uint64_t>(64ull * sps, (total + wj - 1) / wj);
    }
    std::vector<Seg> &segs = ctx.segs;
    std::vector<size_t> &first_seg = ctx.first_seg;
    first_seg.assign(streams.size() + 1, 0);
    for (size_t i = 0; i < streams.size(); i++) {
        first_seg[i] = segs.size();
        StreamDesc &sd = streams[i];
        sd.cr_out = sd.cr_in; sd.final_pos = 0; sd.incomplete = false;
        if (planned) {
            int64_t prev = 0;
            for (int64_t c : cuts[i]) { segs.push_back(Seg{(uint32_t)i, prev, c}); prev = c; }
            segs.push_back(Seg{(uint32_t)i, prev, (int64_t)sd.len});
            continue;
        }
        uint64_t n = 1;
        if (segmenting && sd.len > seg + seg / 2) n = (sd.len + seg - 1) / seg;
        for (uint64_t k = 0; k < n; k++)
            segs.push_back(Seg{(uint32_t)i, (int64_t)(k * seg), (k + 1 == n) ? (int64_t)sd.len : (int64_t)((k + 1) * seg)});
    }
    first_seg[streams.size()] = segs.size();
    if (segs.empty()) return 0;
    env.note_plan(planned, segs.size());

    std::vector<Job> &jobs = ctx.jobs;
    jobs.assign(segs.size(), Job{});
    ctx.decoupled = segmenting && !balanced && env.decoupled(jobs.size());

    uint64_t max_span = 0;
    for (size_t k = 0; k < segs.size(); k++) {
        const StreamDesc &sd = streams[segs[k].stream];
        Job &j = jobs[k];
        j = walk_job(sd, Cursor{segs[k].b0, (k == first_seg[segs[k].stream]) ? sd.cr_in : env.ctor_cr()}, segs[k].b1, false);
        const bool has_next = k + 1 < segs.size() && segs[k + 1].stream == segs[k].stream;
        static const bool no_tail = getenv("LORA_HIP_NO_TAIL") != nullptr;
        j.probe_limit = (segmenting && has_next && !no_tail && !ctx.decoupled) ? std::min<int64_t>((int64_t)sd.len, segs[k + 1].b1 + 16ll * sps) : 0;
        j.tail_stop_sfd = (j.probe_limit && env.early_probe()) ? 1u : 0u;
        max_span = std::max<uint64_t>(max_span, (uint64_t)(segs[k].b1 - segs[k].b0));
    }
    ctx.rpj1 = recs_for(max_span, sps) + (segmenting ? ctx.rpj2 : 0u);
    ctx.trace_cap = tracing ? (uint32_t)std::min<uint64_t>(2ull * (max_span / sps) + 64ull, 1ull << 22) : 0u;
    env.count_jobs((uint32_t)jobs.size());
    env.set_skip_payload(ctx.decoupled);
    ctx.tp0 = std::chrono::steady_clock::now();
    const int s = env.run_jobs_begin(jobs, ctx.rpj1, ctx.trace_cap, env.run_out(0));
    if (s != 0) return s;
    ctx.launched = true;
    return 0;
}

struct PayloadRound {
    struct Ref { size_t k; uint32_t a; };
    std::vector<Ref> refs;
    std::vector<PayloadReq> reqs;
    bool open = false;
};

template <class Env>
int payload_begin(Env &env, const std::vector<StreamDesc> &streams, const PassCtx &ctx, const RunOut &R1, PayloadRound &pr)
{
    const uint32_t sps = env.sps();
    typedef PayloadRound::Ref Ref;
    std::vector<Ref> &refs = pr.refs;
    std::vector<PayloadReq> &reqs = pr.reqs;
    refs.clear(); reqs.clear(); pr.open = false;
    for (size_t k = 0; k < ctx.jobs.size(); k++) {
        const uint32_t nall = std::min(std::min(R1.res[k].n_attempts, R1.cap), R1.rpj);
        const StreamDesc &sd = streams[ctx.segs[k].stream];
        for (uint32_t a = 0; a < nall; a++) {
            const AttemptRec &r = R1.rec(k, a);
            if (r.status != kAttemptHeaderOnly) continue;
            PayloadReq q{};
            std::memcpy(&q.sk, r.frame, sizeof q.sk);
            q.n_walk = (uint32_t)(q.sk.payload_symbols > 0 ? q.sk.payload_symbols : 1);
            q.stream_off = sd.off; q.stream_len = sd.len;
            q.start = r.end_pos - (int64_t)q.n_walk * (int64_t)sps;
            q.hdr_pos = r.hdr_pos; q.cr_prev = r.cr_prev;
            refs.push_back(Ref{k, a});
            reqs.push_back(q);
        }
    }
    if (reqs.empty()) return 0;
    pr.open = true;
    return env.run_payload_begin(reqs);
}

template <class Env>
int payload_end(Env &env, const std::vector<StreamDesc> &streams, PassCtx &ctx, RunOut &R1, PayloadRound &pr)
{
    if (!pr.open) return 0;
    pr.open = false;
    typedef PayloadRound::Ref Ref;
    std::vector<Ref> &refs = pr.refs;
    std::vector<PayloadReq> &reqs = pr.reqs;
    int s = env.run_payload_end(reqs);
    if (s != 0) return s < 0 ? s : -1;

    struct Plan { std::vector<uint32_t> split; int term = -1; uint32_t term_kind = 0; };
    std::vector<Plan> plan(ctx.jobs.size());
    uint32_t n_moved = 0, n_rerun = 0, n_pending = 0;
    for (size_t i = 0; i < reqs.size(); i++) {
        const size_t k = refs[i].k;
        Plan &pl = plan[k];
        if (pl.term >= 0) continue;
        AttemptRec &r = R1.recs[k * R1.rpj + refs[i].a];
        const PayloadReq &q = reqs[i];
        if (q.status == kPayloadDecoded) {
            r.status = kAttemptFrame;
            r.frame_len = q.frame_len;
            std::memcpy(r.frame, q.frame, std::min<size_t>(q.frame_len, sizeof r.frame));
            r.n_symbols += q.n_walk;
            r.end_pos += q.end_shift;
            if (q.end_shift != 0) { pl.split.push_back(refs[i].a); n_moved++; }
        } else {
            pl.term = (int)refs[i].a; pl.term_kind = q.status == kPayloadOutOfData ? 1u : 2u;
            if (pl.term_kind == 1u) n_pending++; else n_rerun++;
        }
    }
    env.count_payload((uint32_t)reqs.size(), n_moved, n_rerun);
    if (n_moved == 0 && n_rerun == 0 && n_pending == 0) return 0;

    std::vector<Job> rjobs;
    for (size_t k = 0; k < plan.size(); k++) {
        if (plan[k].term < 0 || plan[k].term_kind != 2u) continue;
        const AttemptRec &r = R1.rec(k, (uint32_t)plan[k].term);
        Job j = ctx.jobs[k];
        j.start = r.hdr_pos; j.start_at_header = 1; j.cr_prev = r.cr_prev;
        rjobs.push_back(j);
    }
    RunOut &R3 = env.run_out(1);
    R3.res.clear(); R3.recs.clear();
    if (!rjobs.empty()) {
        env.set_skip_payload(false);
        s = env.run_jobs(rjobs, ctx.rpj1, 0, R3);
        if (s != 0) return s;
    }

    struct Row { JobResult res; std::vector<AttemptRec> recs; };
    std::vector<Seg> nsegs;
    std::vector<Job> njobs;
    std::vector<Row> nrows;
    std::vector<size_t> nfirst(streams.size() + 1, 0);
    size_t rq = 0;
    for (size_t i = 0; i < streams.size(); i++) {
        nfirst[i] = nsegs.size();
        for (size_t k = ctx.first_seg[i]; k < ctx.first_seg[i + 1]; k++) {
            const Plan &pl = plan[k];
            const JobResult &jr = R1.res[k];
            const uint32_t n_rows = std::min(std::min(jr.n_attempts + (jr.tail_valid ? jr.tail_n_attempts : 0u), R1.cap), R1.rpj);
            uint32_t lo = 0;
            int64_t b0 = ctx.segs[k].b0;
            std::vector<uint32_t> cuts;
            for (uint32_t a : pl.split) if (pl.term < 0 || (int)a < pl.term) cuts.push_back(a);
            for (size_t c = 0; c <= cuts.size(); c++) {
                const bool last = c == cuts.size();
                Row row;
                Job j = ctx.jobs[k];
                Seg sg = ctx.segs[k];
                j.start = b0; sg.b0 = b0;
                if (!last) {
                    const uint32_t hi = cuts[c];
                    const AttemptRec &e = R1.rec(k, hi);
                    int32_t shift = 0;
                    for (size_t t = 0; t < reqs.size(); t++) if (refs[t].k == k && refs[t].a == hi) shift = reqs[t].end_shift;
                    const int64_t assumed_end = e.end_pos - shift;
                    for (uint32_t a = lo; a <= hi; a++) row.recs.push_back(R1.rec(k, a));
                    row.res = JobResult{};
                    row.res.final_pos = e.end_pos; row.res.n_attempts = hi - lo + 1u; row.res.final_cr = (uint32_t)e.frame[1] >> 5;
                    row.res.stop_reason = 0; row.res.pad = 0; row.res.npush = 0; row.res.tail_valid = 0;
                    j.scan_limit = assumed_end; j.probe_limit = 0; j.tail_stop_sfd = 0;
                    sg.b1 = assumed_end;
                    b0 = assumed_end; lo = hi + 1u;
                } else if (pl.term >= 0 && pl.term_kind == 1u) {
                    const uint32_t hi = (uint32_t)pl.term;
                    for (uint32_t a = lo; a <= hi; a++) row.recs.push_back(R1.rec(k, a));
                    AttemptRec &e = row.recs.back();
                    e.status = kAttemptOutOfData; e.frame_len = 0;
                    row.res = JobResult{};
                    row.res.final_pos = e.start_pos; row.res.n_attempts = hi - lo + 1u; row.res.final_cr = (uint32_t)e.frame[1] >> 5;
                    row.res.stop_reason = 1; row.res.pad = 1; row.res.npush = 0; row.res.tail_valid = 0;
// ... 13 lines not shown
                        if (nr.pad && nr.n_attempts == 1u) nr.final_pos = old.start_pos;
                    }
                    nr.n_attempts += hi - lo;
                    nr.tail_first_rec += hi - lo;
                    row.res = nr;
                    rq++;
                } else {
                    for (uint32_t a = lo; a < n_rows; a++) row.recs.push_back(R1.rec(k, a));
                    row.res = jr;
                    row.res.n_attempts = jr.n_attempts >= lo ? jr.n_attempts - lo : 0u;
                    row.res.tail_first_rec = jr.tail_first_rec >= lo ? jr.tail_first_rec - lo : 0u;
                }
                nsegs.push_back(sg);
                njobs.push_back(j);
                nrows.push_back(std::move(row));
            }
        }
    }
    nfirst[streams.size()] = nsegs.size();
    uint32_t stride = 1;
    for (const Row &r : nrows) stride = std::max<uint32_t>(stride, (uint32_t)r.recs.size());
    R1.res.resize(nrows.size());
    R1.recs.resize_uninit(nrows.size() * (size_t)stride);
    R1.rpj = stride; R1.cap = std::max(R1.cap, stride);
    for (size_t k = 0; k < nrows.size(); k++) {
        R1.res[k] = nrows[k].res;
        for (size_t a = 0; a < nrows[k].recs.size(); a++) R1.recs[k * stride + a] = nrows[k].recs[a];
    }
    ctx.segs.swap(nsegs); ctx.jobs.swap(njobs); ctx.first_seg.swap(nfirst);
    return 1;
}


struct Probe {
    uint32_t stream; size_t target; Cursor start; int job; int tail_of;
    const RunOut *rep_out; size_t rep_job;
};

struct ProbePlan {
    std::vector<Probe> probes;
    std::vector<size_t> first_probe;
    std::vector<Job> jobs;
    uint32_t rpj = 0;
};

template <class Env>
int rerun_wrong_branch(Env &env, const std::vector<StreamDesc> &streams, const PassCtx &ctx, RunOut &R1)
{
    std::vector<Job> rjobs;
    std::vector<size_t> rk;
    for (size_t i = 0; i < streams.size(); i++) {
        for (size_t k = ctx.first_seg[i] + 1; k < ctx.first_seg[i + 1]; k++) {
            const AttemptRec *L = tail_probe_last(R1, k - 1);
            if (!L || (L->status != kAttemptAtHeader && L->status != kAttemptAtSfd)) continue;
            const bool at_sfd = L->status == kAttemptAtSfd;
            if (at_sfd && L->n_sfd == 0u) continue;
            const int a = find_record(R1, k, [&](const AttemptRec &r) {
                return header_bearing(r, true) && (at_sfd ? passed_sfd_state(r, L->sfd_pos[L->n_sfd - 1u], L->sfd_fails[L->n_sfd - 1u]) : r.hdr_pos == L->hdr_pos);
            });
            if (a < 0 || !wrong_fec_branch(R1.rec(k, (uint32_t)a), L->cr_prev)) continue;
            Job j = ctx.jobs[k];
            j.cr_prev = L->cr_prev;
            rjobs.push_back(j);
            rk.push_back(k);
        }
    }
    if (rjobs.empty()) return 0;
    RunOut &R3 = env.run_out(1);
    R3.res.clear(); R3.recs.clear();
    env.count_slow_path();
    env.set_skip_payload(ctx.decoupled);
    const int s = env.run_jobs(rjobs, ctx.rpj1, 0, R3);
    if (s != 0) return s;
    for (size_t q = 0; q < rk.size(); q++) {
        const JobResult &nr = R3.res[q];
        const uint32_t n = nr.n_attempts + (nr.tail_valid ? nr.tail_n_attempts : 0u);
        if (n > R1.rpj || n > R3.cap) continue;
        R1.res[rk[q]] = nr;
        for (uint32_t a = 0; a < n; a++) R1.recs[rk[q] * R1.rpj + a] = R3.rec(q, a);
    }
    if (debug_on()) fprintf(stderr, "[lora_hip] %zu segment job(s) run again with the header FEC branch their predecessor's tail probe reported\n", rjobs.size());
    return 0;
}

inline bool plan_repair(const PassCtx &ctx, const RunOut &R1, const StreamDesc &sd, const AttemptRec &L, Probe &pb, std::vector<Job> &launch,
                        const RunOut &out)
{
    if (L.status != kAttemptAtHeader || L.hdr_pos < 0) return false;
    if (any_segment_record(R1, ctx.first_seg[pb.stream], pb.target, [&](const AttemptRec &r) { return r.hdr_pos == L.hdr_pos; })) return false;
    const Job &target = ctx.jobs[pb.target];
    Job j = walk_job(sd, Cursor{L.hdr_pos, L.cr_prev}, target.scan_limit, false);
    j.start_at_header = 1; j.probe_limit = target.probe_limit;
    pb.rep_out = &out;
    pb.rep_job = launch.size();
    launch.push_back(j);
    return true;
}

inline void plan_probes(uint32_t sps, const std::vector<StreamDesc> &streams, const PassCtx &ctx, const RunOut &R1, const RunOut &R2, bool repair,
                        ProbePlan &plan)
{
    const std::vector<Seg> &segs = ctx.segs;
    std::vector<Probe> &probes = plan.probes;
    probes.clear(); plan.jobs.clear();
    plan.first_probe.assign(streams.size() + 1, 0);
    auto has_header = [&](size_t k) { return find_record(R1, k, [](const AttemptRec &r) { return header_bearing(r, true); }) >= 0; };
    auto job_ok = [&](size_t k) { return !R1.res[k].pad && R1.res[k].stop_reason != 2u; };
    for (size_t i = 0; i < streams.size(); i++) {
        plan.first_probe[i] = probes.size();
        const size_t f = ctx.first_seg[i], e = ctx.first_seg[i + 1];
        if (e - f < 2) continue;
        const StreamDesc &sd = streams[i];
        bool chain = job_ok(f), pending = false;
        Cursor cur{R1.res[f].final_pos, R1.res[f].final_cr};
        size_t cur_job = f;
        auto add_probe = [&](size_t target, int64_t limit) {
            const bool tail = R1.res[cur_job].tail_valid && ctx.jobs[cur_job].probe_limit == limit;
            probes.push_back(Probe{(uint32_t)i, target, cur, tail ? -1 : (int)plan.jobs.size(), tail ? (int)cur_job : -1, nullptr, 0});
            if (!tail) plan.jobs.push_back(walk_job(sd, cur, limit, true));
        };
        for (size_t k = f + 1; k < e && chain; k++) {
            if (cur.pos >= segs[k].b1) continue;
            if (!has_header(k)) { pending = true; continue; }
            add_probe(k, std::min<int64_t>((int64_t)sd.len, segs[k].b1 + 16ll * sps));
            chain = job_ok(k);
            cur = Cursor{R1.res[k].final_pos, R1.res[k].final_cr};
            cur_job = k;
            pending = false;
        }
        if (chain && pending) add_probe(e - 1, (int64_t)sd.len);
    }
    plan.first_probe[streams.size()] = probes.size();
    bool through = false;
    for (Probe &pb : probes) {
        if (pb.job >= 0) continue;
        const AttemptRec *L = tail_probe_last(R1, (size_t)pb.tail_of);
        if (!L || L->status != kAttemptAtSfd || L->n_sfd == 0u) continue;
        const int64_t pos = L->sfd_pos[L->n_sfd - 1u];
        const uint32_t fails = L->sfd_fails[L->n_sfd - 1u];
        if (any_segment_record(R1, ctx.first_seg[pb.stream], pb.target, [&](const AttemptRec &r) { return passed_sfd_state(r, pos, fails); })) continue;
        Job j = walk_job(streams[pb.stream], pb.start, ctx.jobs[(size_t)pb.tail_of].probe_limit, true);
        if (repair) {
            j.scan_limit = ctx.jobs[pb.target].scan_limit; j.stop_at_header = 0;
            through = true;
        }
        pb.job = (int)plan.jobs.size(); pb.tail_of = -1;
        plan.jobs.push_back(j);
    }
    plan.rpj = through ? std::max(ctx.rpj2, ctx.rpj1) : ctx.rpj2;
    if (!repair) return;
    for (Probe &pb : probes) {
        if (pb.job >= 0) continue;
        const AttemptRec *L = tail_probe_last(R1, (size_t)pb.tail_of);
        if (L && plan_repair(ctx, R1, streams[pb.stream], *L, pb, plan.jobs, R2)) plan.rpj = std::max(plan.rpj, ctx.rpj1);
    }
}

template <class Env>
int repair_explicit_probes(Env &env, const std::vector<StreamDesc> &streams, const PassCtx &ctx, const RunOut &R1, const RunOut &R2, ProbePlan &plan,
                           RunOut &R4)
{
    std::vector<Job> rjobs;
    for (Probe &pb : plan.probes) {
        if (pb.job < 0) continue;
        const size_t pj = (size_t)pb.job;
        if (!plan.jobs[pj].stop_at_header) continue;
        const JobResult &pr = R2.res[pj];
        if (!pr.pad || pr.n_attempts == 0u || pr.n_attempts > R2.cap) continue;
        plan_repair(ctx, R1, streams[pb.stream], R2.rec(pj, pr.n_attempts - 1u), pb, rjobs, R4);
    }
    if (rjobs.empty()) return 0;
    env.count_probes((uint32_t)rjobs.size());
    return env.run_jobs(rjobs, ctx.rpj1, 0, R4);
}

struct ProbeView {
    JobResult res; const AttemptRec *recs; uint32_t cap; int64_t limit;
    uint32_t n_done() const
    {
        const uint32_t n = res.pad ? res.n_attempts - 1u : res.n_attempts;
        return n < cap ? n : cap;
    }
};

inline std::vector<ProbeView> probe_views(const PassCtx &ctx, const RunOut &R1, const RunOut &R2, const ProbePlan &plan)
{
    std::vector<ProbeView> pv(plan.probes.size());
    for (size_t q = 0; q < plan.probes.size(); q++) {
        const Probe &pb = plan.probes[q];
        ProbeView &v = pv[q];
        if (pb.job >= 0) {
            const size_t pj = (size_t)pb.job;
            v.res = R2.res[pj]; v.recs = R2.recs.data() + pj * R2.rpj; v.cap = R2.cap; v.limit = plan.jobs[pj].scan_limit;
// ... 26 lines not shown
    sd.pwr.apply(jr.npush, jr.push_tail);
    return true;
}

template <class Env>
int stitch_stream(Env &env, StreamDesc &sd, size_t i, const PassCtx &ctx, const RunOut &R1, const ProbePlan &plan, const std::vector<ProbeView> &pv)
{
    const uint32_t sps = env.sps();
    const std::vector<Seg> &segs = ctx.segs;
    const size_t f = ctx.first_seg[i];
    sd.scan_pos = segs[f].b0; sd.scan_pwr = sd.pwr;
    const bool first_known = end_known(R1, f);
    for (uint32_t a = 0; first_known && a < R1.n_done(f); a++) adopt(env, R1.rec(f, a), sd);
    if (ctx.tracing) env.append_trace(R1, (uint32_t)f, ctx.trace_cap, sd.abs_base);
    Cursor cur = first_known ? end_cursor(R1, f) : Cursor{segs[f].b0, sd.cr_in};
    int64_t covered = first_known ? segs[f].b1 : segs[f].b0;
    if (first_known && R1.res[f].pad) sd.incomplete = true;
    else if (first_known) sd.pwr.apply(R1.res[f].npush, R1.res[f].push_tail);
    auto serial_to = [&](int64_t limit, const char *why) -> int {
        if (debug_on()) fprintf(stderr, "[lora_hip] serial fallback stream %u pos %lld -> %lld: %s\n", sd.id, (long long)cur.pos, (long long)limit, why);
        env.count_slow_path();
        int r = run_serial(env, sd, cur, limit, false);
        covered = std::max(covered, limit);
        return r;
    };
    if (!first_known) {
        if (const int r = serial_to(segs[f].b1, "first segment's pending record did not fit")) return r;
    } else if (!sd.incomplete && R1.res[f].stop_reason == 2u)
        if (const int r = serial_to(segs[f].b1, "first segment out of records")) return r;
    for (size_t q = plan.first_probe[i]; q < plan.first_probe[i + 1] && !sd.incomplete; q++) {
        const Probe &pb = plan.probes[q];
        const int64_t b1 = segs[pb.target].b1;
        if (cur.pos >= b1) continue;
        if (pb.start.pos != cur.pos || pb.start.cr != cur.cr) {
            if (const int r = serial_to(b1, "probe start differs from the true state")) return r;
            continue;
        }
        const ProbeView &view = pv[q];
        const JobResult &pr = view.res;
        if (pr.pad && pr.n_attempts > view.cap) {
            if (const int r = serial_to(b1, "probe out of records")) return r;
            continue;
        }
        for (uint32_t a = 0; a < view.n_done(); a++) adopt(env, view.recs[a], sd);
        if (!pr.pad) {
            cur = Cursor{pr.final_pos, pr.final_cr};
            sd.pwr.apply(pr.npush, pr.push_tail);
            covered = std::max(covered, std::min<int64_t>(view.limit, b1));
            if (pr.stop_reason == 2u || (cur.pos < b1 && cur.pos + 2 * (int64_t)sps <= (int64_t)sd.len))
                if (const int r = serial_to(b1, "probe ended without a header")) return r;
            continue;
        }
        const AttemptRec &L = view.recs[pr.n_attempts - 1u];
        if (L.status != kAttemptAtHeader && L.status != kAttemptAtSfd) {
            cur = Cursor{L.start_pos, L.cr_prev};
            sd.incomplete = true;
            break;
        }
        const bool at_sfd = L.status == kAttemptAtSfd;
        const int64_t probe_sfd_pos = (at_sfd && L.n_sfd) ? L.sfd_pos[L.n_sfd - 1u] : -1;
        const uint32_t probe_sfd_fails = (at_sfd && L.n_sfd) ? L.sfd_fails[L.n_sfd - 1u] : 0u;
        int match = -1;
        size_t mk = 0;
        for (size_t k = f + 1; k <= pb.target && match < 0; k++) {
            if (segs[k].b1 <= cur.pos) continue;
            mk = k;
            match = find_record(R1, k, [&](const AttemptRec &r) {
                return header_bearing(r, false) && (at_sfd ? passed_sfd_state(r, probe_sfd_pos, probe_sfd_fails) : r.hdr_pos == L.hdr_pos) &&
                       !wrong_fec_branch(r, L.cr_prev);
            });
            if (match >= 0 && !end_known(R1, k)) match = -1;
        }
        if (match < 0 && pb.rep_out && !at_sfd) {
            const RunOut &RR = *pb.rep_out;
            const size_t rj = pb.rep_job;
            if (RR.n_done(rj) >= 1u && RR.rec(rj, 0).hdr_pos == L.hdr_pos && RR.res[rj].stop_reason != 2u && end_known(RR, rj)) {
                if (!adopt_from_header(env, sd, cur, L, RR, rj, 0, false)) break;
                covered = std::max(covered, b1);
                env.count_repair();
                continue;
            }
        }
        if (match < 0) {
            if (debug_on()) {
                fprintf(stderr, "[lora_hip] probe for segment %zu [%lld, %lld): start %lld cr %u -> trig %lld hdr %lld (stopped %s, FIND_SFD state %lld / %u)\n", pb.target, (long long)segs[pb.target].b0, (long long)b1,
                        (long long)pb.start.pos, pb.start.cr, (long long)L.trig_pos, (long long)L.hdr_pos, at_sfd ? "behind its first FIND_SFD step" : "at the header", (long long)probe_sfd_pos, probe_sfd_fails);
                for (size_t k = pb.target ? pb.target - 1 : 0; k <= pb.target; k++)
                    for (uint32_t a = 0; a < std::min(R1.res[k].n_attempts, R1.cap); a++) {
                        const AttemptRec &r = R1.rec(k, a);
                        fprintf(stderr, "[lora_hip]    job %zu [%lld, %lld) rec %u status %u start %lld trig %lld hdr %lld end %lld\n", k, (long long)segs[k].b0, (long long)segs[k].b1, a, r.status,
                                (long long)r.start_pos, (long long)r.trig_pos, (long long)r.hdr_pos, (long long)r.end_pos);
                    }
            }
            cur = Cursor{L.start_pos, L.cr_prev};
            if (const int r = serial_to(b1, at_sfd ? "no segment job passed through the probe's FIND_SFD state" : "no segment job entered the same header")) return r;
            continue;
        }
        if (R1.rec(mk, (uint32_t)match).status == kAttemptOutOfData) {
            cur = Cursor{L.start_pos, L.cr_prev};
            sd.incomplete = true;
            break;
        }
        if (!adopt_from_header(env, sd, cur, L, R1, mk, (uint32_t)match, true)) break;
        covered = std::max(covered, segs[mk].b1);
        if (R1.res[mk].stop_reason == 2u)
            if (const int r = serial_to(segs[mk].b1, "segment job out of records")) return r;
    }
    if (!sd.incomplete && cur.pos < (int64_t)sd.len && covered < (int64_t)sd.len && cur.pos + 2 * (int64_t)sps <= (int64_t)sd.len)
        if (const int r = serial_to((int64_t)sd.len, "uncovered tail")) return r;
    if (sd.incomplete) {
        cur.pos = sd.scan_pos;
        sd.pwr = sd.scan_pwr;
    }
    sd.final_pos = cur.pos;
    sd.cr_out = cur.cr;
    return 0;
}

template <class Env>
int decode_end(Env &env, std::vector<StreamDesc> &streams, PassCtx &ctx)
{
    if (!ctx.launched) return 0;
    ctx.launched = false;
    RunOut &R1 = env.run_out(0), &R2 = env.run_out(1);
    int s = env.run_jobs_end(R1);
    if (s != 0) return s;
    const auto tp1 = std::chrono::steady_clock::now();
    if (debug_jobs_on())
        for (size_t k = 0; k < ctx.jobs.size(); k++) dump_job("job", k, ctx.jobs[k], R1);
    if (ctx.segmenting) {
        s = rerun_wrong_branch(env, streams, ctx, R1);
        if (s != 0) return s;
    }
    PayloadRound pround;
    struct PayloadGuard { Env &env; bool armed; ~PayloadGuard() { if (armed) env.abort_payload(); } } pguard{env, false};
    if (ctx.decoupled) {
        pguard.armed = true;
        s = payload_begin(env, streams, ctx, R1, pround);
        if (s != 0) return s;
        pguard.armed = pround.open;
    }
    env.set_skip_payload(false);
    static const bool no_repair = getenv("LORA_HIP_NO_REPAIR") != nullptr;
    const bool repair = !ctx.tracing && !no_repair;
    ProbePlan plan;
    while (true) {
        plan_probes(env.sps(), streams, ctx, R1, R2, repair, plan);
        R2.res.clear(); R2.recs.clear();
// ... 46 lines not shown
```

gr_lora_amd/csrc/lora_walker2.inc.hip:

```cpp

constexpr int kW2DetectK = 4;
#ifndef LORA_W2_WAVES_SF7
#define LORA_W2_WAVES_SF7 8
#endif
#ifndef LORA_W2_WAVES_SF8
#define LORA_W2_WAVES_SF8 8
#endif
#ifndef LORA_W2_SFD_K
#define LORA_W2_SFD_K 2
#endif
#ifndef LORA_W2_EU_SF8
#define LORA_W2_EU_SF8 4
#endif
constexpr int kW2MaxWaves = LORA_W2_WAVES_SF7 > LORA_W2_WAVES_SF8 ? LORA_W2_WAVES_SF7 : LORA_W2_WAVES_SF8;

constexpr int kW2SfdK = LORA_W2_SFD_K;

enum W2Mode : int32_t { kPlanExit = 0, kPlanDetect, kPlanSync, kPlanSfd, kPlanPause, kPlanDecode, kPlanFinalize };

struct alignas(16) W2Plan {
    int64_t pos;
    int32_t mode;
    int32_t buf;
    int32_t resolve_prev;
    int32_t n_win;
    int32_t prev_n;
    int32_t zmode;
};

struct alignas(16) W2State {
    int64_t  pos, att_start, att_trig, att_hdr;
    int32_t  state, done, stop_reason, in_attempt;
    uint32_t corr_fails, cr, has_crc, payload_length;
    int32_t  payload_symbols;
    uint32_t n_words, n_cw, n_sym;
    uint32_t n_att, npush, n_steps, frame_ok;
    uint32_t att_cr_prev, att_ambig;
    float    energy_threshold;
    float    push_tail[4];
    uint8_t  phdr[4];
    uint32_t fin_pending, fin_n_bytes, fin_plen;
    int32_t  fin_st, fin_consumed, fin_bin, fin_fine;
};

struct alignas(16) W2Stats {
    long long prev_t;
    int32_t   prev_state;
    uint32_t  cyc[6], rounds[6], ctl[4];
};

struct alignas(16) W2Shared {
    float    red[kW2MaxWaves * 72 + 8];
    float    specf[kW2MaxWaves][4];
    float    detf[kW2MaxWaves * kW2DetectK][4];
    int32_t  detn[kW2MaxWaves];
    int32_t  speci[2][kW2MaxWaves][4];
    W2Plan   plan[2];
    Shared   sh;
    W2State  st;
    W2Stats  stats;
    int64_t  ph_start;
    uint32_t ph_go, ph_cr, ph_natt, ph_pad;
    uint32_t det_streak;
    uint32_t prio;
    uint32_t words_pk[2];
    strict::Cands sc;
    uint32_t words_pk16[4];
};

struct W2Tabs {
    const float  *v;
    const float  *dd;
    float        *scratch;
};

template <int WAVES>
__device__ __forceinline__ void w2_block_argmax_first(float &v, int &idx, float *red)
{
    const int lane = threadIdx.x & 63, wave = threadIdx.x >> 6;
#pragma unroll
    for (int o = 32; o > 0; o >>= 1) {
        const float ov = __shfl_xor(v, o, 64);
        const int oi = __shfl_xor(idx, o, 64);
        if (ov > v || (ov == v && oi < idx)) { v = ov; idx = oi; }
    }
    __syncthreads();
    if (lane == 0) { red[wave] = v; ((int *)red)[16 + wave] = idx; }
    __syncthreads();
    v = red[0]; idx = ((int *)red)[16];
#pragma unroll
    for (int w = 1; w < WAVES; w++) {
        const float ov = red[w];
        const int oi = ((int *)red)[16 + w];
        if (ov > v || (ov == v && oi < idx)) { v = ov; idx = oi; }
    }
}

__device__ __forceinline__ bool w2_pre_step(W2State &S, const Job &job, uint32_t rec_cap, uint32_t sps)
{
    if (S.state == kDetect && !S.in_attempt) {
        if (S.pos >= job.scan_limit) { S.stop_reason = 0; S.done = 1; return false; }
        if (S.n_att >= rec_cap) { S.stop_reason = 2; S.done = 1; return false; }
        if (job.max_attempts && S.n_att >= job.max_attempts) { S.stop_reason = 3; S.done = 1; return false; }
    }
    if (S.pos + 2 * (int64_t)sps > (int64_t)job.stream_len) { S.stop_reason = 1; S.done = 1; return false; }
    return true;
}

template <bool KEEP_SFD = false>
__device__ __forceinline__ void w2_end_step(W2State &S, const Job &job, const LaunchCfg &C, AttemptRec *recs, StepRec *trace, int32_t st_in,
                            int32_t consumed, int32_t step_bin, int32_t fine, float step_val, long long t_start, bool lead = true)
{
    if (trace && lead && S.n_steps < C.trace_cap) {
        StepRec &s = trace[S.n_steps];
        s.state = st_in; s.consumed = consumed; s.pos = S.pos; s.bin = step_bin; s.fine = fine; s.value = step_val;
// ... 391 lines not shown
    const uint32_t jid = blockIdx.x;
    if (jid >= C.n_jobs) return;
    Job job = C.jobs[jid];
    if constexpr (SF == 7) job = uniform_job(job);
    uint32_t rec_cap = C.recs_per_job;
    const float2 *__restrict__ X = C.iq + job.stream_off;
    const int64_t n_items = (int64_t)job.stream_len;
    AttemptRec *recs = C.recs + (size_t)jid * C.recs_per_job;
    StepRec *trace = C.trace ? C.trace + (size_t)jid * C.trace_cap : nullptr;
    const int wave = threadIdx.x >> 6, lane = threadIdx.x & 63;
    const bool is_ctl = wave == kW2Workers;
    const bool t0 = threadIdx.x == kW2Workers * 64;
    if (is_ctl) __builtin_amdgcn_s_setprio(2);

    const uint32_t dbg_t0 = (uint32_t)__builtin_amdgcn_s_memrealtime(), dbg_c0 = (uint32_t)(clock64() >> 6);
    WaveTabs FT{};
    if constexpr (GRAD) {
        for (uint32_t i = threadIdx.x; i < 3u * sps + 40u; i += kW2) vl[i] = P.up_ifreq_v[i];
        FT.v = vl;
    } else {
        if constexpr (LD == 3 && SF >= 7) FT = wave_tabs_to_lds<SF>(P, tab2, vl, kW2);
        else FT = wave_tabs_to_lds_d<SF, LD>(P, tab2, vl, kW2);
    }
    for (uint32_t i = threadIdx.x; i < sps; i += kW2) ddl[i] = P.down_ifreq[i] - P.down_ifreq_avg;

    auto plan_from = [&](W2State &S, W2Plan &pl, bool zreq = false ) {
        pl.buf = 0; pl.resolve_prev = 0; pl.n_win = kW2Workers; pl.pos = S.pos; pl.prev_n = 0; pl.zmode = zreq ? 1 : 0;
        if (!S.done) (void)w2_pre_step(S, job, rec_cap, sps);
        if (S.done) { pl.mode = kPlanExit; return; }
        if (S.fin_pending) { pl.mode = kPlanFinalize; return; }
        if (S.state != kDetect) W.det_streak = 0u;
        switch (S.state) {
        case kDetect:
            pl.mode = kPlanDetect; pl.n_win = W.det_streak++ == 0u ? 1 : kW2DetectK;
            return;
        case kSync: pl.mode = kPlanSync; break;
        case kFindSfd: pl.mode = kPlanSfd; break;
        case kPause: pl.mode = kPlanPause; break;
        default:
            pl.mode = kPlanDecode; pl.n_win = kW2Win;
            if (S.state == kDecodePayload && !P.implicit) {
                const int32_t rem = S.payload_symbols - (int32_t)S.n_words;
                pl.n_win = rem < kW2Win ? (rem > 0 ? rem : 1) : kW2Win;
            }
            break;
        }
    };
    auto plan_from_state = [&](W2Plan &pl) { plan_from(S, pl); };

    W2Tabs T{vl, ddl, W.red};
    uint32_t *bal_mine = nullptr, *bal_other = nullptr;
    uint32_t bal_rem = 0xffffffffu, bal_seen = 0u, bal_slot = 0u;
    if (t0) W.prio = 0u;
    if (t0 && C.balance) {
        const uint32_t hw = __builtin_amdgcn_s_getreg((31 << 11) | 4), xcc = __builtin_amdgcn_s_getreg((31 << 11) | 20);
        const uint32_t cu = ((xcc & 7u) << 8) | ((hw >> 8) & 0xffu);
        bal_slot = atomicAdd(&C.balance[2u * kBalanceCus + cu], 1u) & 1u;
        bal_mine = C.balance + 2u * cu + bal_slot;
        bal_other = C.balance + 2u * cu + (bal_slot ^ 1u);
    }
    for (int phase = 0; phase < 2; phase++) {
    if (t0) {
        S = W2State{};
        S.state = kDetect; S.pos = job.start; S.cr = job.cr_prev; S.has_crc = P.ctor_crc;
        S.phdr[1] = (uint8_t)((P.ctor_cr << 5) | (P.ctor_crc << 4));
        S.att_start = job.start; S.att_trig = -1; S.att_hdr = -1; S.att_cr_prev = job.cr_prev;
        if (job.start_at_header && phase == 0) { S.state = kDecodeHeader; S.in_attempt = 1; S.att_trig = job.start; S.att_hdr = job.start; }
        if (phase == 0) W.stats = W2Stats{};
        W.stats.prev_state = -1;
        W.det_streak = 0u;
        plan_from_state(W.plan[0]);
    }

    for (uint32_t it = 0;; it++) {
        __syncthreads();
        const W2Plan &pl_in = W.plan[it & 1u];
        const uint64_t pl_pp = (uint64_t)pl_in.pos;
        const int64_t plan_pos = (int64_t)(((uint64_t)__builtin_amdgcn_readfirstlane((uint32_t)(pl_pp >> 32)) << 32) | __builtin_amdgcn_readfirstlane((uint32_t)pl_pp));
        const int32_t plan_mode = __builtin_amdgcn_readfirstlane(pl_in.mode), plan_buf = __builtin_amdgcn_readfirstlane(pl_in.buf);
        const int32_t plan_resolve_prev = __builtin_amdgcn_readfirstlane(pl_in.resolve_prev), plan_n_win = __builtin_amdgcn_readfirstlane(pl_in.n_win);
        const int32_t plan_prev_n = __builtin_amdgcn_readfirstlane(pl_in.prev_n), plan_z = __builtin_amdgcn_readfirstlane(pl_in.zmode);
        W2Plan &next = W.plan[(it + 1u) & 1u];
        if (plan_mode == kPlanExit) break;
        const int64_t pos = plan_pos;
        const long long t_start = clock64();
        if (t0) {
            W2Stats &Q = W.stats;
            const int sidx = plan_mode == kPlanDetect ? 0 : plan_mode == kPlanSync ? 1 : plan_mode == kPlanSfd ? 2 : plan_mode == kPlanPause ? 3 : 5;
            if (Q.prev_state >= 0) { Q.cyc[Q.prev_state] += (uint32_t)((t_start - Q.prev_t) >> 6); Q.rounds[Q.prev_state]++; }
            Q.prev_state = sidx; Q.prev_t = t_start;
        }
        if (t0 && bal_mine) {
            W.prio = (bal_rem > bal_seen || (bal_rem == bal_seen && bal_slot != 0u)) ? 1u : 0u;
            const int64_t target = phase == 0 ? job.scan_limit + (job.probe_limit > job.scan_limit ? 12 * (int64_t)sps : 0) : pos + 6 * (int64_t)sps;
            const int64_t left = (target - pos) / (int64_t)sps;
            bal_rem = left < 1 ? 1u : (left > 0x3fffffff ? 0x3fffffffu : (uint32_t)left);
            __hip_atomic_store(bal_mine, bal_rem, __ATOMIC_RELAXED, __HIP_MEMORY_SCOPE_AGENT);
            bal_seen = __hip_atomic_load(bal_other, __ATOMIC_RELAXED, __HIP_MEMORY_SCOPE_AGENT);
        }
        if (!is_ctl) {
            if (W.prio) __builtin_amdgcn_s_setprio(1); else __builtin_amdgcn_s_setprio(0);
        }
        const int64_t wpos = pos + (int64_t)wave * sps;

        if (plan_mode == kPlanDetect) {
            const int kd = plan_n_win;
// ... 81 lines not shown
                }
            }
            continue;
        }

        if (plan_mode == kPlanSync) {
            const float2 *__restrict__ x = X + pos;
            if (P.strict_sync) {
                w2_sync_exact_ifreq<GSF, WAVES>(x, f2);
            } else {
                constexpr int NI = (2 * SPS + kW2 - 1) / kW2;
                float2 xb[NI], xa[NI];
#pragma unroll
                for (int k = 0; k < NI; k++) {
                    const uint32_t i = 1u + threadIdx.x + (uint32_t)k * kW2;
                    if (i < 2u * sps) { xb[k] = x[i - 1]; xa[k] = x[i]; }
                }
                __builtin_amdgcn_sched_group_barrier(0x020, 2 * NI, 0);
                __builtin_amdgcn_sched_group_barrier(0x002, 64 * NI, 0);
#pragma unroll
                for (int k = 0; k < NI; k++) {
                    const uint32_t i = 1u + threadIdx.x + (uint32_t)k * kW2;
                    if (i < 2u * sps) f2[i - 1] = ifreq_prod_z(xb[k], xa[k]);
                }
            }
            __syncthreads();
            if (t0) { f2[2u * sps - 1u] = f2[2u * sps - 2u]; strict::cands_reset(W.sc); }
            __syncthreads();
            float bv, b2;
            int bi, i2;
            w2_sync_closed_form<GSF, WAVES>(f2, pre, P.sync_a, P.sync_b, bv, bi, b2, i2);
            const float my_bv = bv;
            const int my_bi = bi;
            w2_block_argmax_first<WAVES>(bv, bi, W.red);
            if (P.strict_sync) {
                strict::cands_push(W.sc, bv, my_bv, my_bi, b2, i2);
                __syncthreads();
                const int nc = W.sc.n;
                if (nc >= 2 && nc <= strict::kK) {
                    float ev;
                    if constexpr (SF == 7 && LD == 3) bi = strict::resolve_lds_inl<kW2>(f2, SPS, vl, &W.sc, reinterpret_cast<float *>(pre), 1024, &ev);
                    else bi = strict::resolve_lds<kW2>(f2, SPS, vl, &W.sc, reinterpret_cast<float *>(pre), 1024, &ev);
                    bv = ev;
                }
            }
            if (t0) {
                const int32_t consumed = (bi == 0x7fffffff) ? 0 : bi;
                W2State L = S;
                L.state = kFindSfd;
                w2_end_step(L, job, C, recs, trace, kSync, consumed, -1, 0, bv, t_start);
                W2Plan np;
                plan_from(L, np);
                next = np; S = L;
            }
            if constexpr (ALIAS) {
                __syncthreads();
                const v2f *__restrict__ src = reinterpret_cast<const v2f *>(P.wave_tabs);
                for (uint32_t i = threadIdx.x; i < NENT; i += kW2) tab2[i] = src[i];
            }
            continue;
        }

        if (plan_mode == kPlanSfd) {
            constexpr int kSfdWin = kW2SfdK * kW2Workers;
            static_assert(kW2SfdK <= 2 && kSfdWin <= 64, "results go to specf[w][k] / speci[k][w]");
#pragma unroll
            for (int k = 0; k < kW2SfdK; k++) {
                const int64_t kpos = wpos + (int64_t)k * kW2Workers * sps;
                const bool kvalid = !is_ctl && wave < plan_n_win && kpos + 2 * (int64_t)sps <= n_items;
                float c = 0.0f;
                int32_t fine = 0;
                int32_t pz = 0;
                if (kvalid) {
                    const W2SfdOut r = plan_z ? w2_sfd_window_zm<GSF, (4 << LD)>(X + kpos, T.v, T.dd, T.scratch + wave * 72, P.down_ifreq_sd, P.down_ifreq_dsum, P.sync_a, P.sync_b)
                                              : w2_sfd_window<GSF, false, (4 << LD)>(X + kpos, T.v, T.dd, T.scratch + wave * 72, P.down_ifreq_sd, P.down_ifreq_dsum, P.sync_a, P.sync_b);
                    c = r.c; fine = r.fine; pz = r.pz;
                }
                if (lane == 0 && !is_ctl) { W.specf[wave][k] = c; W.speci[k][wave][0] = kvalid ? 1 : 0; W.speci[k][wave][1] = fine; W.speci[k][wave][2] = pz; }
            }
            __syncthreads();
            if (is_ctl) {
                W2State L = S;
                const int qw = lane % kW2Workers, qk = lane / kW2Workers;
                const float my_c = lane < kSfdWin ? W.specf[qw][qk] : 0.0f;
                const int32_t my_v = lane < kSfdWin ? W.speci[qk][qw][0] : 0, my_f = lane < kSfdWin ? W.speci[qk][qw][1] : 0;
                const int32_t my_p = lane < kSfdWin ? W.speci[qk][qw][2] : 0;
                asm volatile("s_waitcnt lgkmcnt(0)" ::: "memory");
                bool zreq = false;
                for (int w = 0; w < kSfdWin; w++) {
                    if (w > 0 && !w2_pre_step(L, job, rec_cap, sps)) break;
                    if (!__builtin_amdgcn_readlane(my_v, w)) break;
                    if (__builtin_amdgcn_readlane(my_p, w)) { zreq = true; break; }
                    const float cw = __builtin_bit_cast(float, __builtin_amdgcn_readlane(__builtin_bit_cast(int32_t, my_c), w));
                    int32_t fw = 0;
                    if (cw > 0.96f) {
                        L.state = kPause;
                    } else {
                        if (cw < -0.97f) fw = __builtin_amdgcn_readlane(my_f, w);
                        else L.corr_fails++;
                        if (L.corr_fails > 4u) L.state = kDetect;
                    }
                    w2_end_step(L, job, C, recs, trace, kFindSfd, (int32_t)sps + fw, -1, fw, cw, t_start, t0);
                    if (L.state != kFindSfd || L.done || fw != 0) break;
                }
                if (L.state == kPause && !L.done && w2_pre_step(L, job, rec_cap, sps)) {
                    L.state = kDecodeHeader;
// ... 135 lines not shown
            const long long tr2 = clock64();
            W2Plan np;
            if (predicted) {
                int32_t n_next = kW2Win;
                if (L.state == kDecodePayload && !P.implicit) {
                    const int32_t rem = L.payload_symbols - (int32_t)L.n_words - dn;
                    n_next = rem < kW2Win ? (rem > 0 ? rem : 0) : kW2Win;
                }
                np.mode = kPlanDecode; np.pos = dpos + (int64_t)dn * sps; np.buf = plan_buf ^ 1; np.resolve_prev = 1; np.n_win = n_next;
                np.prev_n = dn; np.zmode = 0;
            } else {
                plan_from(L, np, zreq);
            }
            const long long tr3 = clock64();
            if (t0) {
                next = np;
                S = L;
                if constexpr (W16) { W.words_pk16[0] = wpk[0]; W.words_pk16[1] = wpk[1]; W.words_pk16[2] = wpk[2]; W.words_pk16[3] = wpk[3]; }
                else { W.words_pk[0] = wpk[0]; W.words_pk[1] = wpk[1]; }
                asm volatile("s_waitcnt lgkmcnt(0)" ::: "memory");
                W.stats.ctl[0] += (uint32_t)((tr1 - tr0) >> 6); W.stats.ctl[1] += (uint32_t)((tr2 - tr1) >> 6); W.stats.ctl[2] += (uint32_t)((tr3 - tr2) >> 6);
                W.stats.ctl[3] += (uint32_t)((clock64() - tr3) >> 6);
                W.stats.cyc[4] += (uint32_t)((clock64() - tr0) >> 6); W.stats.rounds[4]++;
            }
        }
    }

    __syncthreads();
    if (t0) {
        const bool in_attempt = S.in_attempt != 0;
        if (in_attempt && S.n_att < rec_cap) {
            AttemptRec &r = recs[S.n_att];
            r.status = (S.stop_reason == 3) ? kAttemptAtHeader : kAttemptOutOfData;
            r.start_pos = S.att_start; r.trig_pos = S.att_trig; r.hdr_pos = S.att_hdr; r.end_pos = S.pos;
            r.npush = S.npush;
            for (int i = 0; i < 4; i++) r.push_tail[i] = S.push_tail[i];
            r.cr_prev = S.att_cr_prev; r.hdr_ambig = S.att_ambig; r.n_symbols = S.n_sym; r.frame_len = 0; r.n_sfd = 0;
        }
        JobResult &jr = C.results[jid];
        const int64_t e_pos = in_attempt ? S.att_start : S.pos;
        const uint32_t e_natt = S.n_att + (in_attempt ? 1u : 0u), e_npush = in_attempt ? 0u : S.npush, e_pad = in_attempt ? 1u : 0u;
        bool go = false;
        if (phase == 0) {
            jr.final_pos = e_pos;
            jr.n_attempts = e_natt;
            jr.final_cr = S.cr;
            jr.npush = e_npush;
            for (int i = 0; i < 4; i++) jr.push_tail[i] = S.push_tail[i];
            jr.stop_reason = (uint32_t)S.stop_reason;
            jr.n_steps = S.n_steps < C.trace_cap ? S.n_steps : C.trace_cap;
            jr.pad = e_pad;
            jr.tail_valid = 0;
            go = job.probe_limit > job.scan_limit && S.stop_reason == 0 && !in_attempt && !trace && e_natt < C.recs_per_job;
            W.ph_go = go ? 1u : 0u; W.ph_start = e_pos; W.ph_cr = S.cr; W.ph_natt = e_natt; W.ph_pad = 0;
        } else {
            jr.tail_valid = 1; jr.tail_first_rec = W.ph_natt;
            jr.tail_final_pos = e_pos; jr.tail_n_attempts = e_natt; jr.tail_final_cr = S.cr; jr.tail_npush = e_npush;
            for (int i = 0; i < 4; i++) jr.tail_push_tail[i] = S.push_tail[i];
            jr.tail_stop_reason = (uint32_t)S.stop_reason; jr.tail_pad = e_pad; jr.tail_rsv = 0;
        }
        if (!go) {
            W2Stats &Q = W.stats;
            if (Q.prev_state >= 0) { Q.cyc[Q.prev_state] += (uint32_t)((clock64() - Q.prev_t) >> 6); Q.rounds[Q.prev_state]++; }
            for (int i = 0; i < 6; i++) { jr.cyc[i] = Q.cyc[i]; jr.rounds[i] = Q.rounds[i]; }
            for (int i = 0; i < 4; i++) jr.ctl[i] = Q.ctl[i];
            jr.dbg[0] = __builtin_amdgcn_s_getreg((31 << 11) | 4); jr.dbg[1] = __builtin_amdgcn_s_getreg((31 << 11) | 20);
            jr.dbg[2] = dbg_t0; jr.dbg[3] = (uint32_t)__builtin_amdgcn_s_memrealtime();
            jr.dbg[4] = dbg_c0; jr.dbg[5] = (uint32_t)(clock64() >> 6);
        }
    }
    if (phase == 1) break;
    __syncthreads();
    if (!W.ph_go) break;
    bal_rem = 0xffffffffu;
    {
        const int64_t st = W.ph_start;
        const uint32_t lo = __builtin_amdgcn_readfirstlane((uint32_t)st), hi = __builtin_amdgcn_readfirstlane((uint32_t)((uint64_t)st >> 32));
        const uint32_t natt = __builtin_amdgcn_readfirstlane(W.ph_natt);
        job.start = (int64_t)(((uint64_t)hi << 32) | lo);
        job.cr_prev = __builtin_amdgcn_readfirstlane(W.ph_cr);
        job.scan_limit = job.probe_limit; job.stop_at_header = 1; job.max_attempts = 0;
        recs += natt;
        rec_cap = C.recs_per_job - natt;
    }
    __syncthreads();
    }
    if (t0 && bal_mine) __hip_atomic_store(bal_mine, 0u, __ATOMIC_RELAXED, __HIP_MEMORY_SCOPE_AGENT);
}

constexpr int kW2WavesSf7 = LORA_W2_WAVES_SF7, kW2WavesSf8 = LORA_W2_WAVES_SF8;
__global__ __launch_bounds__(64 * kW2WavesSf7, 4) void walker2_kernel_sf7(DevParams P, LaunchCfg C) { walker2_body<7, kW2WavesSf7, false>(P, C); }
__global__ __launch_bounds__(64 * kW2WavesSf8, LORA_W2_EU_SF8) void walker2_kernel_sf8(DevParams P, LaunchCfg C) { walker2_body<8, kW2WavesSf8, false>(P, C); }
__global__ __launch_bounds__(64 * kW2WavesSf8, 2) void walker2_kernel_sf8_wide(DevParams P, LaunchCfg C) { walker2_body<8, kW2WavesSf8, false>(P, C); }
__global__ __launch_bounds__(64 * kW2WavesSf7, 2) void walker2_kernel_sf7_wide(DevParams P, LaunchCfg C) { walker2_body<7, kW2WavesSf7, false>(P, C); }
__global__ __launch_bounds__(64 * kW2WavesSf7, 2) void walker2_kernel_sf7_grad_wide(DevParams P, LaunchCfg C) { walker2_body<7, kW2WavesSf7, true>(P, C); }
__global__ __launch_bounds__(64 * kW2WavesSf8, 2) void walker2_kernel_sf8_grad_wide(DevParams P, LaunchCfg C) { walker2_body<8, kW2WavesSf8, true>(P, C); }
#ifndef LORA_W2_EU_GRAD_SF7
#define LORA_W2_EU_GRAD_SF7 4
#endif
#ifndef LORA_W2_EU_GRAD_SF8
#define LORA_W2_EU_GRAD_SF8 4
#endif
__global__ __launch_bounds__(64 * kW2WavesSf7, LORA_W2_EU_GRAD_SF7) void walker2_kernel_sf7_grad(DevParams P, LaunchCfg C) { walker2_body<7, kW2WavesSf7, true>(P, C); }
__global__ __launch_bounds__(64 * kW2WavesSf8, LORA_W2_EU_GRAD_SF8) void walker2_kernel_sf8_grad(DevParams P, LaunchCfg C) { walker2_body<8, kW2WavesSf8, true>(P, C); }
__global__ __launch_bounds__(64 * kW2WavesSf7, 4) void walker2_kernel_sf7_skip(DevParams P, LaunchCfg C) { walker2_body<7, kW2WavesSf7, false, true>(P, C); }
__global__ __launch_bounds__(64 * kW2WavesSf8, 2) void walker2_kernel_sf8_skip(DevParams P, LaunchCfg C) { walker2_body<8, kW2WavesSf8, false, true>(P, C); }
__global__ __launch_bounds__(64 * kW2WavesSf7, LORA_W2_EU_GRAD_SF7) void walker2_kernel_sf7_grad_skip(DevParams P, LaunchCfg C) { walker2_body<7, kW2WavesSf7, true, true>(P, C); }
// ... 31 lines not shown
```

include/lora_hip.h:

```cpp
#ifndef LORA_HIP_H
#define LORA_HIP_H

#include <stddef.h>
#include <stdint.h>

#ifdef __cplusplus
extern "C" {
#endif

#define LORA_HIP_ABI_VERSION 4

typedef enum lora_hip_status {
    LORA_HIP_OK = 0,
    LORA_HIP_ERR_BAD_SF = -1,
    LORA_HIP_ERR_BAD_CONFIG = -2,
    LORA_HIP_ERR_NO_DEVICE = -3,
    LORA_HIP_ERR_HIP = -4,
    LORA_HIP_ERR_NOMEM = -5,
    LORA_HIP_ERR_ARG = -6,
    LORA_HIP_ERR_OVERFLOW = -7,
    LORA_HIP_ERR_INTERNAL = -8
} lora_hip_status;

typedef enum lora_hip_iq_format {
// ... 103 lines not shown
lora_hip_status lora_hip_mux_work(lora_hip_mux_t *m, uint32_t channel, const float *iq, size_t n_items);
lora_hip_status lora_hip_mux_flush(lora_hip_mux_t *m);
lora_hip_status lora_hip_mux_set_latency(lora_hip_mux_t *m, float max_latency_ms);
lora_hip_status lora_hip_mux_set_max_ahead(lora_hip_mux_t *m, size_t max_ahead_items);
size_t          lora_hip_mux_frames_available(const lora_hip_mux_t *m);
lora_hip_status lora_hip_mux_poll_frame(lora_hip_mux_t *m, uint8_t *buf, size_t cap, size_t *len, lora_hip_frame_info_t *info);
lora_hip_status lora_hip_mux_passes(const lora_hip_mux_t *m, uint64_t *passes, uint64_t *passes_by_latency);
const char     *lora_hip_mux_last_error(const lora_hip_mux_t *m);

lora_hip_status lora_hip_decode_device(lora_hip_decoder_t *h, const void *d_iq, size_t total_items,
                                       const uint64_t *stream_off, const uint64_t *stream_len,
                                       uint32_t n_streams, void *hip_stream);

lora_hip_status lora_hip_iq_unpack_device(int device, const void *d_raw, size_t n_items, int fmt, float scale, void *d_out_cf32,
                                          void *hip_stream);

#define LORA_HIP_BEGIN_IQ_READY 1u
lora_hip_status lora_hip_decode_device_begin(lora_hip_decoder_t *h, const void *d_iq, size_t total_items,
                                             const uint64_t *stream_off, const uint64_t *stream_len,
                                             uint32_t n_streams, void *hip_stream, uint32_t flags);
lora_hip_status lora_hip_decode_device_end(lora_hip_decoder_t *h);
lora_hip_status lora_hip_decode_device_prepass(lora_hip_decoder_t *h, const void *d_iq, size_t total_items,
                                               const uint64_t *stream_off, const uint64_t *stream_len,
                                               uint32_t n_streams, void *hip_stream, uint32_t flags);

lora_hip_status lora_hip_gap_starts_device(lora_hip_decoder_t *h, const void *d_iq, size_t total_items,
                                           const uint64_t *stream_off, const uint64_t *stream_len, uint32_t n_streams,
                                           int64_t *pos, size_t cap, uint32_t *counts, void *hip_stream);

size_t          lora_hip_frames_available(const lora_hip_decoder_t *h);
lora_hip_status lora_hip_poll_frame(lora_hip_decoder_t *h, uint8_t *buf, size_t cap, size_t *len,
                                    lora_hip_frame_info_t *info);

lora_hip_status lora_hip_drain_frames(lora_hip_decoder_t *h, uint8_t *buf, size_t cap, lora_hip_frame_info_t *infos,
                                      size_t max_frames, size_t *n_frames);

lora_hip_status lora_hip_drain_slots(lora_hip_decoder_t *h, uint8_t *slots, size_t slot_bytes, size_t max_slots,
                                     size_t *n_frames);

lora_hip_status lora_hip_demod_symbols_device(lora_hip_decoder_t *h, const void *d_iq, size_t total_items,
                                              const int64_t *offsets, size_t n, int demod,
                                              uint32_t *bins_out, void *hip_stream);

lora_hip_status lora_hip_demod_symbols_ex_device(lora_hip_decoder_t *h, const void *d_iq, size_t total_items,
                                                 const int64_t *offsets, size_t n, int demod,
                                                 uint32_t *bins_out, int32_t *fine_out, void *hip_stream);

lora_hip_status lora_hip_last_timing(const lora_hip_decoder_t *h, lora_hip_timing_t *t);
const char     *lora_hip_walker_kernel_name(const lora_hip_decoder_t *h);
lora_hip_status lora_hip_last_payload_pass(const lora_hip_decoder_t *h, uint32_t *packets, uint32_t *moved, uint32_t *rerun, uint32_t *rounds,
                                           uint32_t *symbols, float *ms);

lora_hip_status lora_hip_last_plan(const lora_hip_decoder_t *h, uint32_t *burst_aware, uint32_t *segments);
lora_hip_status lora_hip_get_table(const lora_hip_decoder_t *h, int which, float *buf, size_t cap_floats, size_t *n_floats);
size_t          lora_hip_trace(const lora_hip_decoder_t *h, const lora_hip_step_t **steps);
void            lora_hip_trace_clear(lora_hip_decoder_t *h);

lora_hip_status lora_hip_estimate_cfo_device(lora_hip_decoder_t *h, const void *d_iq, size_t total_items,
                                             const int64_t *offsets, size_t n, int mode, float *cfo_hz_out,
                                             void *hip_stream);

lora_hip_status lora_hip_ref_ifreq_device(lora_hip_decoder_t *h, const void *d_iq, size_t n_items, float *arg_out, float *ifreq_out,
                                          void *hip_stream);

typedef struct lora_hip_window_stats {
    int32_t bin_down; float peak_down, total_down;
    int32_t bin_up;   float peak_up, total_up;
} lora_hip_window_stats_t;
lora_hip_status lora_hip_window_stats_device(lora_hip_decoder_t *h, const void *d_iq, size_t total_items, const int64_t *offsets,
                                             size_t n, lora_hip_window_stats_t *out, void *hip_stream);
typedef struct lora_hip_preamble {
    int64_t  header_pos;
    int64_t  run_pos;
    uint32_t stream;
    uint32_t run_len;
    int32_t  bin;
    int32_t  sfd_index;
    float    pmr;
    float    cfo_bins, cfo_hz;
    int32_t  delta;
} lora_hip_preamble_t;
lora_hip_status lora_hip_detect_preambles_device(lora_hip_decoder_t *h, const void *d_iq, size_t total_items,
                                                 const uint64_t *stream_off, const uint64_t *stream_len, uint32_t n_streams,
                                                 float threshold, lora_hip_preamble_t *out, size_t cap, size_t *n_found,
                                                 void *hip_stream);

lora_hip_status lora_hip_decode_at_headers_device(lora_hip_decoder_t *h, const void *d_iq, size_t total_items,
                                                  const uint64_t *stream_off, const uint64_t *stream_len, uint32_t n_streams,
                                                  const lora_hip_preamble_t *pre, size_t n, void *hip_stream);

typedef struct lora_hip_frame_check {
    uint8_t  has_header;
    uint8_t  header_checksum_ok;
    uint8_t  has_crc;
    uint8_t  crc_ok;
    uint8_t  header_checksum_rx, header_checksum_calc;
    uint16_t crc_rx, crc_calc;
    uint16_t reserved;
} lora_hip_frame_check_t;
lora_hip_status lora_hip_check_frame(const uint8_t *blob, size_t len, lora_hip_frame_check_t *out);

#ifdef __cplusplus
}
#endif
#endif
```

Baseline: 262,500.

## Stop tail probes early at SYNC when successor segment job left SYNC identically

Adds a cross-job handoff in the fast walker kernel. Each segment job records, in a device buffer, the position where its first attempt leaves SYNC. A tail probe of the previous segment stops as soon as it leaves SYNC at that same position, instead of walking on to the SFD or header. The host stitcher then treats these sync stops as merge points with the successor's first record. This cuts redundant tail-probe walking, at the cost of double-buffered atomic position arrays, extra memsets and more complex stitching logic.

```diff
diff --git a/gr_lora_amd/capi.py b/gr_lora_amd/capi.py
--- a/gr_lora_amd/capi.py
+++ b/gr_lora_amd/capi.py
@@ -20,7 +20,7 @@
     "lora_hip_abi_version", "lora_hip_strerror", "lora_hip_last_error", "lora_hip_create", "lora_hip_destroy",
     "lora_hip_get_geometry", "lora_hip_set_sf", "lora_hip_set_samp_rate", "lora_hip_work", "lora_hip_flush",
     "lora_hip_decode_device", "lora_hip_frames_available", "lora_hip_poll_frame", "lora_hip_drain_frames", "lora_hip_drain_slots", "lora_hip_demod_symbols_device", "lora_hip_demod_symbols_ex_device",
-    "lora_hip_last_timing", "lora_hip_last_plan", "lora_hip_get_table", "lora_hip_last_payload_pass", "lora_hip_gap_starts_device", "lora_hip_decode_device_begin", "lora_hip_decode_device_end", "lora_hip_decode_device_prepass", "lora_hip_trace", "lora_hip_trace_clear", "lora_hip_check_frame", "lora_hip_estimate_cfo_device", "lora_hip_ref_ifreq_device",
+    "lora_hip_last_timing", "lora_hip_last_plan", "lora_hip_last_sync_stops", "lora_hip_get_table", "lora_hip_last_payload_pass", "lora_hip_gap_starts_device", "lora_hip_decode_device_begin", "lora_hip_decode_device_end", "lora_hip_decode_device_prepass", "lora_hip_trace", "lora_hip_trace_clear", "lora_hip_check_frame", "lora_hip_estimate_cfo_device", "lora_hip_ref_ifreq_device",
     "lora_hip_set_stream_latency", "lora_hip_stream_info", "lora_hip_stream_info_ex", "lora_hip_walker_kernel_name", "lora_hip_window_stats_device", "lora_hip_detect_preambles_device", "lora_hip_decode_at_headers_device",
     "lora_hip_mux_create", "lora_hip_mux_destroy", "lora_hip_mux_work", "lora_hip_mux_flush", "lora_hip_mux_set_latency", "lora_hip_mux_set_max_ahead", "lora_hip_mux_frames_available",
     "lora_hip_mux_poll_frame", "lora_hip_mux_passes", "lora_hip_mux_last_error",
@@ -251,6 +251,8 @@
     L.lora_hip_demod_symbols_ex_device.argtypes = [vp, vp, C.c_size_t, vp, C.c_size_t, C.c_int, vp, vp, vp]
     L.lora_hip_last_timing.argtypes = [vp, C.POINTER(Timing)]
     L.lora_hip_last_plan.argtypes = [vp, C.POINTER(C.c_uint32), C.POINTER(C.c_uint32)]
+    if hasattr(L, "lora_hip_last_sync_stops") or not os.environ.get("LORA_HIP_LIB"):
+        L.lora_hip_last_sync_stops.argtypes = [vp, C.POINTER(C.c_uint32), C.POINTER(C.c_uint32)]
     L.lora_hip_last_payload_pass.argtypes = [vp, C.POINTER(C.c_uint32), C.POINTER(C.c_uint32), C.POINTER(C.c_uint32), C.POINTER(C.c_uint32), C.POINTER(C.c_uint32), C.POINTER(C.c_float)]
     L.lora_hip_decode_device_begin.argtypes = [vp, vp, C.c_size_t, vp, vp, C.c_uint32, vp, C.c_uint32]
     L.lora_hip_decode_device_end.argtypes = [vp]
@@ -696,6 +698,11 @@
         self._check(self.L.lora_hip_last_plan(self.h, C.byref(b), C.byref(n)))
         return bool(b.value), int(n.value)
 
+    def sync_stops(self):
+        t, s = C.c_uint32(0), C.c_uint32(0)
+        self._check(self.L.lora_hip_last_sync_stops(self.h, C.byref(t), C.byref(s)))
+        return int(t.value), int(s.value)
+
     def table(self, which: int) -> np.ndarray:
         n = C.c_size_t()
         self._check(self.L.lora_hip_get_table(self.h, which, None, 0, C.byref(n)))
diff --git a/gr_lora_amd/csrc/lora_device.h b/gr_lora_amd/csrc/lora_device.h
--- a/gr_lora_amd/csrc/lora_device.h
+++ b/gr_lora_amd/csrc/lora_device.h
@@ -75,6 +75,7 @@
     int64_t  probe_limit;
     uint32_t start_at_header;
     uint32_t tail_stop_sfd;
+    uint32_t sync_succ;
 };
 
 struct AttemptRec {
@@ -113,6 +114,8 @@
     uint32_t dbg[6];
 };
 
+constexpr uint32_t kStopAtSync = 4;
+
 struct StepRec {
     int32_t  state, consumed;
     int64_t  pos;
@@ -135,6 +138,8 @@
     uint32_t n_jobs;
     uint32_t *balance;
     uint32_t skip_payload;
+    unsigned long long *sync_pos;
+    unsigned long long *sync_clear;
 };
 constexpr uint32_t kBalanceCus = 2048;
 constexpr uint32_t kBalanceWords = 3u * kBalanceCus;
@@ -173,6 +178,7 @@
     uint8_t  frame[kMaxFrame + 4];
 };
 int launch_payload_chain(const DevParams &p, const uint32_t *d_bins, const int32_t *d_fine, const DemodAlt &alt, const PayloadDesc *descs, PayloadOut *outs, uint32_t n_packets, void *stream);
+bool walker_has_sync_stop(const DevParams &p);
 bool walker_has_skip_variant(const DevParams &p);
 int launch_ref_ifreq(const float2 *x, uint32_t n, float *d_arg, float *d_ifreq, void *stream);
 int launch_cfo(const DevParams &p, const float2 *iq, const int64_t *d_offsets, uint32_t n, int mode, float *d_out, void *stream);
diff --git a/gr_lora_amd/csrc/lora_kernels.hip b/gr_lora_amd/csrc/lora_kernels.hip
--- a/gr_lora_amd/csrc/lora_kernels.hip
+++ b/gr_lora_amd/csrc/lora_kernels.hip
@@ -367,7 +367,7 @@
     u.start = (int64_t)uni64((uint64_t)j.start); u.scan_limit = (int64_t)uni64((uint64_t)j.scan_limit);
     u.stream_id = uni32(j.stream_id); u.cr_prev = uni32(j.cr_prev); u.max_attempts = uni32(j.max_attempts); u.stop_at_header = uni32(j.stop_at_header);
     u.probe_limit = (int64_t)uni64((uint64_t)j.probe_limit);
-    u.start_at_header = uni32(j.start_at_header); u.tail_stop_sfd = uni32(j.tail_stop_sfd);
+    u.start_at_header = uni32(j.start_at_header); u.tail_stop_sfd = uni32(j.tail_stop_sfd); u.sync_succ = uni32(j.sync_succ);
     return u;
 }
 
@@ -981,6 +981,7 @@
 }
 
 bool walker_has_skip_variant(const DevParams &p) { return (use_w3_kernel(p) || use_fast_kernel(p)) && !p.implicit; }
+bool walker_has_sync_stop(const DevParams &p) { return use_fast_kernel(p); }
 
 static WalkerKernel pick_walker(const DevParams &p, bool half = false, bool skip = false)
 {
diff --git a/gr_lora_amd/csrc/lora_runtime.cpp b/gr_lora_amd/csrc/lora_runtime.cpp
--- a/gr_lora_amd/csrc/lora_runtime.cpp
+++ b/gr_lora_amd/csrc/lora_runtime.cpp
@@ -138,7 +138,7 @@
     hipEvent_t ev0 = nullptr, ev1 = nullptr, ev_done = nullptr;
     hipEvent_t ev_pre0 = nullptr, ev_pre1 = nullptr, ev_dep = nullptr;
     hipStream_t pre_stream = nullptr;
-    struct Pending { uint32_t nj = 0, recs_per_job = 0, eager = 0, trace_cap = 0; bool direct = true, open = false; hipStream_t st = nullptr;
+    struct Pending { uint32_t nj = 0, recs_per_job = 0, eager = 0, trace_cap = 0; bool direct = true, open = false, main = false; hipStream_t st = nullptr;
                      std::chrono::steady_clock::time_point hp0, hp1; } pending;
     PassCtx pass;
     std::vector<StreamDesc> pass_streams;
@@ -157,6 +157,11 @@
     PinnedBuf<JobResult> p_res;
     PinnedBuf<AttemptRec> p_recs;
     DevBuf<uint32_t> d_balance;
+    DevBuf<unsigned long long> d_sync[2];
+    uint32_t sync_dirty[2] = {0, 0};
+    int sync_cur = 0;
+    bool sync_next = false;
+    uint32_t last_tail_probes = 0, last_sync_stops = 0;
     DevBuf<float> d_env_E;
     DevBuf<unsigned long long> d_env_buf;
     PinnedBuf<EnvStream> p_env_streams;
@@ -448,6 +453,29 @@
     }
     c.balance = no_balance ? nullptr : h->d_balance.p;
     c.skip_payload = h->launch_skip ? 1u : 0u;
+    static const bool no_sync_stop = getenv("LORA_HIP_NO_SYNC_STOP") != nullptr;
+    const bool main_launch = h->sync_next;
+    h->sync_next = false;
+    h->pending.main = main_launch;
+    bool sync_stop = main_launch && !no_sync_stop && !trace_cap && !h->launch_skip && walker_has_sync_stop(h->P);
+    if (sync_stop) {
+        sync_stop = false;
+        for (const Job &j : jobs) sync_stop = sync_stop || j.sync_succ != 0u;
+    }
+    if (sync_stop) {
+        const int a = h->sync_cur, b = a ^ 1;
+        for (int i = 0; i < 2; i++) {
+            if (h->d_sync[i].cap >= nj) continue;
+            HIP_TRY(h, h->d_sync[i].reserve(nj));
+            HIP_TRY(h, hipMemsetAsync(h->d_sync[i].p, 0, h->d_sync[i].cap * sizeof(unsigned long long), st));
+            h->sync_dirty[i] = 0;
+        }
+        if (h->sync_dirty[a]) HIP_TRY(h, hipMemsetAsync(h->d_sync[a].p, 0, h->sync_dirty[a] * sizeof(unsigned long long), st));
+        c.sync_pos = h->d_sync[a].p; c.sync_clear = h->d_sync[b].p;
+        h->sync_dirty[a] = nj;
+        if (h->sync_dirty[b] <= nj) h->sync_dirty[b] = 0;
+        h->sync_cur = b;
+    }
     HIP_TRY(h, hipEventRecord(h->ev0, st));
     if (nj >= h->last_kernel_jobs) { h->last_kernel = walker_kernel_name_for(h->P, nj, h->launch_skip); h->last_kernel_jobs = nj; }
     if (launch_walker(h->P, c, st) != 0) return fail(h, LORA_HIP_ERR_HIP, "walker launch failed: %s", hipGetErrorString(hipGetLastError()));
@@ -481,14 +509,14 @@
         fprintf(stderr, "[lora_hip] per-job avg kcycles (rounds): DETECT %.0f (%.1f) SYNC %.0f (%.1f) SFD %.0f (%.1f) PAUSE %.0f (%.1f) HDR %.0f (%.1f) PAYLOAD %.0f (%.1f)\n",
                 cyc[0] / nj / 1e3, rnd[0] / nj, cyc[1] / nj / 1e3, rnd[1] / nj, cyc[2] / nj / 1e3, rnd[2] / nj, cyc[3] / nj / 1e3, rnd[3] / nj, cyc[4] / nj / 1e3, rnd[4] / nj, cyc[5] / nj / 1e3, rnd[5] / nj);
         {
-            double na = 0, nt = 0, ntv = 0; uint32_t sr[4] = {0, 0, 0, 0}, tsr[4] = {0, 0, 0, 0}, tpad = 0;
+            double na = 0, nt = 0, ntv = 0; uint32_t sr[4] = {0, 0, 0, 0}, tsr[5] = {0, 0, 0, 0, 0}, tpad = 0;
             for (uint32_t j = 0; j < nj; j++) {
                 const JobResult &r = out.res[j];
                 na += r.n_attempts; sr[r.stop_reason & 3u]++;
-                if (r.tail_valid) { ntv++; nt += r.tail_n_attempts; tsr[r.tail_stop_reason & 3u]++; tpad += r.tail_pad; }
+                if (r.tail_valid) { ntv++; nt += r.tail_n_attempts; tsr[r.tail_stop_reason == kStopAtSync ? 4u : r.tail_stop_reason & 3u]++; tpad += r.tail_pad; }
             }
-            fprintf(stderr, "[lora_hip] attempts/job %.2f, stop reasons %u/%u/%u/%u; tails %.0f (attempts/tail %.2f, stop reasons %u/%u/%u/%u, pending %u)\n", na / nj, sr[0], sr[1],
-                    sr[2], sr[3], ntv, ntv ? nt / ntv : 0.0, tsr[0], tsr[1], tsr[2], tsr[3], tpad);
+            fprintf(stderr, "[lora_hip] attempts/job %.2f, stop reasons %u/%u/%u/%u; tails %.0f (attempts/tail %.2f, stop reasons %u/%u/%u/%u/%u, pending %u)\n", na / nj, sr[0], sr[1],
+                    sr[2], sr[3], ntv, ntv ? nt / ntv : 0.0, tsr[0], tsr[1], tsr[2], tsr[3], tsr[4], tpad);
         }
         double ctl[4] = {0};
         for (uint32_t j = 0; j < nj; j++) for (int i = 0; i < 4; i++) ctl[i] += 64.0 * out.res[j].ctl[i];
@@ -525,9 +553,18 @@
             std::memcpy(&out.recs[(size_t)j * stride + a], src, n);
         }
     }
+    if (h->pending.main) {
+        uint32_t tails = 0, at_sync = 0;
+        for (uint32_t j = 0; j < nj; j++) {
+            const JobResult &r = out.res[j];
+            if (r.tail_valid && r.tail_pad) { tails++; at_sync += r.tail_stop_reason == kStopAtSync ? 1u : 0u; }
+        }
+        h->last_tail_probes = tails; h->last_sync_stops = at_sync;
+    }
     if (dbg_stats && h->P.use_fast) {
-        double sync_rounds = 0; uint32_t frames = 0, tails = 0, early = 0;
+        double sync_rounds = 0; uint32_t frames = 0, tails = 0, early = 0, at_sync = 0;
         for (uint32_t j = 0; j < nj; j++) {
+            at_sync += (out.res[j].tail_valid && out.res[j].tail_pad && out.res[j].tail_stop_reason == kStopAtSync) ? 1u : 0u;
             const JobResult &r = out.res[j];
             sync_rounds += r.rounds[1];
             const uint32_t used = std::min(std::min(eager, max_att), r.n_attempts + (r.tail_valid ? r.tail_n_attempts : 0u));
@@ -537,8 +574,8 @@
                 if (r.tail_valid && a + 1u == r.n_attempts + r.tail_n_attempts && r.tail_pad) { tails++; early += t.status == kAttemptAtSfd ? 1u : 0u; }
             }
         }
-        fprintf(stderr, "[lora_hip] acquisitions: %.0f SYNC rounds for %u frames of this launch (%.2f per frame); %u tail probes reached a packet, %u of them stopped behind their first FIND_SFD step\n",
-                sync_rounds, frames, frames ? sync_rounds / frames : 0.0, tails, early);
+        fprintf(stderr, "[lora_hip] acquisitions: %.0f SYNC rounds for %u frames of this launch (%.2f per frame); %u tail probes reached a packet, %u of them stopped behind their first FIND_SFD step, %u at SYNC\n",
+                sync_rounds, frames, frames ? sync_rounds / frames : 0.0, tails, early, at_sync);
     }
     h->eager_recs = std::min(std::max(max_att, 2u), 8u);
     bool more = false;
@@ -860,6 +897,7 @@
     }
     int run_jobs_begin(const std::vector<Job> &jobs, uint32_t rpj, uint32_t trace_cap, RunOut &out)
     {
+        h->sync_next = true;
         return ::run_jobs_begin(h, d_iq, jobs, rpj, trace_cap, st, out) == LORA_HIP_OK ? 0 : -1;
     }
     int run_jobs_end(RunOut &out) { return ::run_jobs_end(h, out) == LORA_HIP_OK ? 0 : -1; }
@@ -1227,6 +1265,7 @@
     for (int i = 0; i < 2; i++) { h->pipe.dbuf[i].release(); h->feed.stage[i].release(); }
     h->feed.d_raw.release();
     h->p_jobs.release(); h->p_res.release(); h->p_recs.release();
+    h->d_sync[0].release(); h->d_sync[1].release();
     h->d_balance.release(); h->d_env_E.release(); h->d_env_buf.release(); h->p_env_streams.release(); h->p_env_buf.release();
     for (hipEvent_t e : {h->ev0, h->ev1, h->ev_done, h->ev_pre0, h->ev_pre1, h->ev_dep, h->ev_pay0, h->ev_pay1, h->ev_pay_done, h->pipe.up_ev, h->pipe.tail_ev,
                          h->feed.stage_ev[0], h->feed.stage_ev[1]})
@@ -2056,6 +2095,14 @@
     return LORA_HIP_OK;
 }
 
+lora_hip_status lora_hip_last_sync_stops(const lora_hip_decoder_t *h, uint32_t *tail_probes, uint32_t *at_sync)
+{
+    if (!h) return LORA_HIP_ERR_ARG;
+    if (tail_probes) *tail_probes = h->last_tail_probes;
+    if (at_sync) *at_sync = h->last_sync_stops;
+    return LORA_HIP_OK;
+}
+
 lora_hip_status lora_hip_last_payload_pass(const lora_hip_decoder_t *h, uint32_t *packets, uint32_t *moved, uint32_t *rerun, uint32_t *rounds, uint32_t *symbols, float *ms)
 {
     if (!h) return LORA_HIP_ERR_ARG;
diff --git a/gr_lora_amd/csrc/lora_stitch.hpp b/gr_lora_amd/csrc/lora_stitch.hpp
--- a/gr_lora_amd/csrc/lora_stitch.hpp
+++ b/gr_lora_amd/csrc/lora_stitch.hpp
@@ -230,6 +230,16 @@
     if (!jr.tail_valid || !jr.tail_pad || jr.tail_n_attempts == 0u) return nullptr;
     const uint32_t li = std::min(jr.tail_first_rec, R.cap) + jr.tail_n_attempts - 1u;
     return li < R.cap ? &R.rec(k, li) : nullptr;
+}
+
+inline bool tail_at_sync(const RunOut &R, size_t k)
+{
+    const JobResult &jr = R.res[k];
+    return jr.tail_valid && jr.tail_pad && jr.tail_stop_reason == kStopAtSync;
+}
+inline int sync_stop_match(const RunOut &R, size_t succ, bool with_header_only)
+{
+    return (R.res[succ].n_attempts >= 1u && R.cap >= 1u && R.rpj >= 1u && header_bearing(R.rec(succ, 0), with_header_only)) ? 0 : -1;
 }
 
 template <class Pred>
@@ -411,6 +421,7 @@
         static const bool no_tail = getenv("LORA_HIP_NO_TAIL") != nullptr;
         j.probe_limit = (segmenting && has_next && !no_tail && !ctx.decoupled) ? std::min<int64_t>((int64_t)sd.len, segs[k + 1].b1 + 16ll * sps) : 0;
         j.tail_stop_sfd = (j.probe_limit && env.early_probe()) ? 1u : 0u;
+        j.sync_succ = (j.probe_limit && !j.tail_stop_sfd) ? (uint32_t)(k + 2u) : 0u;
         max_span = std::max<uint64_t>(max_span, (uint64_t)(segs[k].b1 - segs[k].b0));
     }
     ctx.rpj1 = recs_for(max_span, sps) + (segmenting ? ctx.rpj2 : 0u);
@@ -500,7 +511,7 @@
         if (plan[k].term < 0 || plan[k].term_kind != 2u) continue;
         const AttemptRec &r = R1.rec(k, (uint32_t)plan[k].term);
         Job j = ctx.jobs[k];
-        j.start = r.hdr_pos; j.start_at_header = 1; j.cr_prev = r.cr_prev;
+        j.start = r.hdr_pos; j.start_at_header = 1; j.cr_prev = r.cr_prev; j.sync_succ = 0;
         rjobs.push_back(j);
     }
     RunOut &R3 = env.run_out(1);
@@ -620,15 +631,16 @@
     for (size_t i = 0; i < streams.size(); i++) {
         for (size_t k = ctx.first_seg[i] + 1; k < ctx.first_seg[i + 1]; k++) {
             const AttemptRec *L = tail_probe_last(R1, k - 1);
-            if (!L || (L->status != kAttemptAtHeader && L->status != kAttemptAtSfd)) continue;
-            const bool at_sfd = L->status == kAttemptAtSfd;
+            const bool at_sync = L && tail_at_sync(R1, k - 1);
+            if (!L || (!at_sync && L->status != kAttemptAtHeader && L->status != kAttemptAtSfd)) continue;
+            const bool at_sfd = !at_sync && L->status == kAttemptAtSfd;
             if (at_sfd && L->n_sfd == 0u) continue;
-            const int a = find_record(R1, k, [&](const AttemptRec &r) {
+            const int a = at_sync ? sync_stop_match(R1, k, true) : find_record(R1, k, [&](const AttemptRec &r) {
                 return header_bearing(r, true) && (at_sfd ? passed_sfd_state(r, L->sfd_pos[L->n_sfd - 1u], L->sfd_fails[L->n_sfd - 1u]) : r.hdr_pos == L->hdr_pos);
             });
             if (a < 0 || !wrong_fec_branch(R1.rec(k, (uint32_t)a), L->cr_prev)) continue;
             Job j = ctx.jobs[k];
-            j.cr_prev = L->cr_prev;
+            j.cr_prev = L->cr_prev; j.sync_succ = 0;
             rjobs.push_back(j);
             rk.push_back(k);
         }
@@ -703,10 +715,15 @@
     for (Probe &pb : probes) {
         if (pb.job >= 0) continue;
         const AttemptRec *L = tail_probe_last(R1, (size_t)pb.tail_of);
-        if (!L || L->status != kAttemptAtSfd || L->n_sfd == 0u) continue;
-        const int64_t pos = L->sfd_pos[L->n_sfd - 1u];
-        const uint32_t fails = L->sfd_fails[L->n_sfd - 1u];
-        if (any_segment_record(R1, ctx.first_seg[pb.stream], pb.target, [&](const AttemptRec &r) { return passed_sfd_state(r, pos, fails); })) continue;
+        if (!L) continue;
+        if (tail_at_sync(R1, (size_t)pb.tail_of)) {
+            if (pb.target == (size_t)pb.tail_of + 1u && sync_stop_match(R1, pb.target, true) >= 0) continue;
+        } else {
+            if (L->status != kAttemptAtSfd || L->n_sfd == 0u) continue;
+            const int64_t pos = L->sfd_pos[L->n_sfd - 1u];
+            const uint32_t fails = L->sfd_fails[L->n_sfd - 1u];
+            if (any_segment_record(R1, ctx.first_seg[pb.stream], pb.target, [&](const AttemptRec &r) { return passed_sfd_state(r, pos, fails); })) continue;
+        }
         Job j = walk_job(streams[pb.stream], pb.start, ctx.jobs[(size_t)pb.tail_of].probe_limit, true);
         if (repair) {
             j.scan_limit = ctx.jobs[pb.target].scan_limit; j.stop_at_header = 0;
@@ -839,7 +856,8 @@
             continue;
         }
         const AttemptRec &L = view.recs[pr.n_attempts - 1u];
-        if (L.status != kAttemptAtHeader && L.status != kAttemptAtSfd) {
+        const bool at_sync = pb.tail_of >= 0 && pr.stop_reason == kStopAtSync;
+        if (!at_sync && L.status != kAttemptAtHeader && L.status != kAttemptAtSfd) {
             cur = Cursor{L.start_pos, L.cr_prev};
             sd.incomplete = true;
             break;
@@ -849,7 +867,12 @@
         const uint32_t probe_sfd_fails = (at_sfd && L.n_sfd) ? L.sfd_fails[L.n_sfd - 1u] : 0u;
         int match = -1;
         size_t mk = 0;
-        for (size_t k = f + 1; k <= pb.target && match < 0; k++) {
+        if (at_sync) {
+            mk = pb.target;
+            if (pb.target == (size_t)pb.tail_of + 1u && segs[mk].b1 > cur.pos) match = sync_stop_match(R1, mk, false);
+            if (match >= 0 && (wrong_fec_branch(R1.rec(mk, (uint32_t)match), L.cr_prev) || !end_known(R1, mk))) match = -1;
+        }
+        for (size_t k = f + 1; !at_sync && k <= pb.target && match < 0; k++) {
             if (segs[k].b1 <= cur.pos) continue;
             mk = k;
             match = find_record(R1, k, [&](const AttemptRec &r) {
@@ -858,7 +881,7 @@
             });
             if (match >= 0 && !end_known(R1, k)) match = -1;
         }
-        if (match < 0 && pb.rep_out && !at_sfd) {
+        if (match < 0 && pb.rep_out && !at_sfd && !at_sync) {
             const RunOut &RR = *pb.rep_out;
             const size_t rj = pb.rep_job;
             if (RR.n_done(rj) >= 1u && RR.rec(rj, 0).hdr_pos == L.hdr_pos && RR.res[rj].stop_reason != 2u && end_known(RR, rj)) {
@@ -871,7 +894,7 @@
         if (match < 0) {
             if (debug_on()) {
                 fprintf(stderr, "[lora_hip] probe for segment %zu [%lld, %lld): start %lld cr %u -> trig %lld hdr %lld (stopped %s, FIND_SFD state %lld / %u)\n", pb.target, (long long)segs[pb.target].b0, (long long)b1,
-                        (long long)pb.start.pos, pb.start.cr, (long long)L.trig_pos, (long long)L.hdr_pos, at_sfd ? "behind its first FIND_SFD step" : "at the header", (long long)probe_sfd_pos, probe_sfd_fails);
+                        (long long)pb.start.pos, pb.start.cr, (long long)L.trig_pos, (long long)L.hdr_pos, at_sync ? "at SYNC" : at_sfd ? "behind its first FIND_SFD step" : "at the header", (long long)(at_sync ? L.end_pos : probe_sfd_pos), probe_sfd_fails);
                 for (size_t k = pb.target ? pb.target - 1 : 0; k <= pb.target; k++)
                     for (uint32_t a = 0; a < std::min(R1.res[k].n_attempts, R1.cap); a++) {
                         const AttemptRec &r = R1.rec(k, a);
@@ -880,7 +903,8 @@
                     }
             }
             cur = Cursor{L.start_pos, L.cr_prev};
-            if (const int r = serial_to(b1, at_sfd ? "no segment job passed through the probe's FIND_SFD state" : "no segment job entered the same header")) return r;
+            if (const int r = serial_to(b1, at_sync ? "the successor's first attempt, which left SYNC where the probe did, is not one to merge with"
+                                                     : at_sfd ? "no segment job passed through the probe's FIND_SFD state" : "no segment job entered the same header")) return r;
             continue;
         }
         if (R1.rec(mk, (uint32_t)match).status == kAttemptOutOfData) {
diff --git a/gr_lora_amd/csrc/lora_walker2.inc.hip b/gr_lora_amd/csrc/lora_walker2.inc.hip
--- a/gr_lora_amd/csrc/lora_walker2.inc.hip
+++ b/gr_lora_amd/csrc/lora_walker2.inc.hip
@@ -60,7 +60,7 @@
     W2State  st;
     W2Stats  stats;
     int64_t  ph_start;
-    uint32_t ph_go, ph_cr, ph_natt, ph_pad;
+    uint32_t ph_go, ph_cr, ph_natt, ph_succ;
     uint32_t det_streak;
     uint32_t prio;
     uint32_t words_pk[2];
@@ -558,6 +558,13 @@
     uint32_t *bal_mine = nullptr, *bal_other = nullptr;
     uint32_t bal_rem = 0xffffffffu, bal_seen = 0u, bal_slot = 0u;
     if (t0) W.prio = 0u;
+    constexpr bool kSyncStop = !SKIP && LD == 3 && (SF == 7 || SF == 8);
+    if constexpr (kSyncStop) {
+        if (t0) {
+            W.ph_succ = (C.sync_pos && job.sync_succ - 1u < C.n_jobs) ? job.sync_succ : 0u;
+            if (C.sync_clear) C.sync_clear[jid] = 0ull;
+        }
+    }
     if (t0 && C.balance) {
         const uint32_t hw = __builtin_amdgcn_s_getreg((31 << 11) | 4), xcc = __builtin_amdgcn_s_getreg((31 << 11) | 20);
         const uint32_t cu = ((xcc & 7u) << 8) | ((hw >> 8) & 0xffu);
@@ -745,6 +752,21 @@
                 W2Plan np;
                 plan_from(L, np);
                 next = np; S = L;
+                if constexpr (kSyncStop) {
+                    if (C.sync_pos && L.n_att == 0u) {
+                        const unsigned long long mine = (unsigned long long)(L.pos + 1);
+                        if (phase == 0) {
+                            if (!job.start_at_header) {
+                                __hip_atomic_store(C.sync_pos + jid, mine, __ATOMIC_RELAXED, __HIP_MEMORY_SCOPE_AGENT);
+                            }
+                        } else {
+                            const uint32_t succ = W.ph_succ;
+                            if (succ != 0u && __hip_atomic_load(C.sync_pos + (succ - 1u), __ATOMIC_RELAXED, __HIP_MEMORY_SCOPE_AGENT) == mine) {
+                                S.stop_reason = (int32_t)kStopAtSync; S.done = 1; next.mode = kPlanExit;
+                            }
+                        }
+                    }
+                }
             }
             if constexpr (ALIAS) {
                 __syncthreads();
@@ -986,7 +1008,7 @@
             jr.pad = e_pad;
             jr.tail_valid = 0;
             go = job.probe_limit > job.scan_limit && S.stop_reason == 0 && !in_attempt && !trace && e_natt < C.recs_per_job;
-            W.ph_go = go ? 1u : 0u; W.ph_start = e_pos; W.ph_cr = S.cr; W.ph_natt = e_natt; W.ph_pad = 0;
+            W.ph_go = go ? 1u : 0u; W.ph_start = e_pos; W.ph_cr = S.cr; W.ph_natt = e_natt;
         } else {
             jr.tail_valid = 1; jr.tail_first_rec = W.ph_natt;
             jr.tail_final_pos = e_pos; jr.tail_n_attempts = e_natt; jr.tail_final_cr = S.cr; jr.tail_npush = e_npush;
diff --git a/include/lora_hip.h b/include/lora_hip.h
--- a/include/lora_hip.h
+++ b/include/lora_hip.h
@@ -179,6 +179,7 @@
                                            uint32_t *symbols, float *ms);
 
 lora_hip_status lora_hip_last_plan(const lora_hip_decoder_t *h, uint32_t *burst_aware, uint32_t *segments);
+lora_hip_status lora_hip_last_sync_stops(const lora_hip_decoder_t *h, uint32_t *tail_probes, uint32_t *at_sync);
 lora_hip_status lora_hip_get_table(const lora_hip_decoder_t *h, int which, float *buf, size_t cap_floats, size_t *n_floats);
 size_t          lora_hip_trace(const lora_hip_decoder_t *h, const lora_hip_step_t **steps);
 void            lora_hip_trace_clear(lora_hip_decoder_t *h);
```

Measured after the change: 267,700 (median of 6 runs). 1.02x the previous value.
